# sota-zk-labs/zkp-implementation

Measured on AMD Instinct MI355X. Metric: G1 MSM scalar-muls/sec, higher is better.
Workload: dtype u32 (unsaturated 28-bit-limb Montgomery, 381-bit Fq; 64-bit accumulate)

## Files before the change

zkp-implementation_amd/build.py:

```python
#!/usr/bin/env python3
import os
import subprocess
import sys

HERE = os.path.dirname(os.path.abspath(__file__))
SRC = os.path.join(HERE, "csrc")
OUT = os.path.join(HERE, "libzkp_hip.so")
SOURCES = ["api.hip", "selftest.hip"]
DEPS = ["api.hip", "ff.hpp", "fq28.hpp", "fq28_inv.hpp", "fr29.hpp", "fr29_mul2_asm.inc", "fq28_mul_asm.inc", "fq28_mul2x_asm.inc", "fq28_sqr_asm.inc", "fq28_mul2_asm.inc", "g1.hpp", "g1_28.hpp", "msm.hpp", "ntt.hpp", "ntt_plan.hpp", "ntt_host.inc", "plonk.hpp",
        "plonk_host.inc", "plonk_compile_host.inc", "ntt_sharded.inc", "fri.hpp", "fri_host.inc", "fri_fr.hpp", "transcript_host.hpp", "pairing_host.hpp", "verify_host.inc", "host_ff.hpp", "kzg_host.hpp", "host_threads.hpp", "knobs.hpp", "msm_plan.hpp", "glv.hpp", "g1_check.hpp", "g1_check_host.inc", "g1_ntt.hpp", "g1_ntt_plan.hpp", "g1_ntt_host.inc", "msm_host.inc", "nova.hpp", "nova_host.inc", "dev_res.hpp", "selftest.hpp", "selftest.hip",
        os.path.join("..", "..", "include", "zkp_hip.h")]


STAMP = OUT + ".srchash"


def source_hash():
    import hashlib
    h = hashlib.sha256()
    for d in DEPS:
        path = os.path.join(SRC, d)
        if os.path.exists(path):
            h.update(d.encode())
            h.update(open(path, "rb").read())
    return h.hexdigest()


def stale():
    if not os.path.exists(OUT) or not os.path.exists(STAMP):
        return True
    return open(STAMP).read().strip() != source_hash()


def build(force=False, verbose=False, defines=(), out=None):
    variant = out is not None
    if not variant and not force and not stale():
        return OUT
    hipcc = os.environ.get("HIPCC", "/opt/rocm/bin/hipcc")
    cmd = [hipcc, "--offload-arch=gfx950", "-O3", "-std=c++17", "-fPIC", "-shared",
           "-Wno-unused-result", "-pthread"] + [f"-D{d}" for d in defines] + [os.path.join(SRC, s) for s in SOURCES] + ["-o", out or OUT]
    if verbose:
        print(" ".join(cmd))
    subprocess.check_call(cmd)
    if not variant:
        with open(STAMP, "w") as f:
            f.write(source_hash())
    return out or OUT


if __name__ == "__main__":
    defs = [a[2:] for a in sys.argv[1:] if a.startswith("-D")]
    outs = [a[2:] for a in sys.argv[1:] if a.startswith("-o")]
    print(build(force="--force" in sys.argv, verbose=True, defines=defs, out=outs[0] if outs else None))
```

zkp-implementation_amd/csrc/api.hip:

```cpp
#include <hip/hip_runtime.h>

#include <algorithm>
#include <array>
#include <atomic>
#include <chrono>
#include <cstdio>
#include <cstdlib>
#include <cstring>
#include <condition_variable>
#include <functional>
#include <map>
#include <memory>
#include <mutex>
#include <new>
#include <string>
#include <thread>
#include <tuple>
#include <type_traits>
#include <vector>

#include "../../include/zkp_hip.h"
#include "host_ff.hpp"
#include "kzg_host.hpp"
#include "msm.hpp"
#include "g1_check.hpp"
#include "ntt.hpp"
#include "g1_ntt.hpp"
#include "plonk.hpp"
#include "nova.hpp"
#include "fri.hpp"
#include "fri_fr.hpp"
#include "selftest.hpp"
#include "transcript_host.hpp"
#include "pairing_host.hpp"

using namespace zkp;
using namespace zkp::host;

namespace {

thread_local std::string g_err;

int fail(int code, const std::string& msg) {
    g_err = msg;
    return code;
}

int on_exception() noexcept {
    try {
        throw;
    } catch (const std::bad_alloc&) {
        try { g_err = "host allocation failed"; } catch (...) {}
        return ZKP_E_NOMEM;
    } catch (const std::exception& e) {
        try { g_err = std::string("internal error: ") + e.what(); } catch (...) {}
        return ZKP_E_DEVICE;
    } catch (...) {
        try { g_err = "internal error: unknown exception"; } catch (...) {}
        return ZKP_E_DEVICE;
    }
}
#define ZKP_CATCH_INT catch (...) { return on_exception(); }

#define HIPCHK(expr)                                                                                        \
    do {                                                                                                    \
        hipError_t e_ = (expr);                                                                             \
        if (e_ != hipSuccess)                                                                               \
            return fail(e_ == hipErrorOutOfMemory ? ZKP_E_NOMEM : ZKP_E_DEVICE,                             \
                        std::string(#expr) + ": " + hipGetErrorString(e_));                                 \
    } while (0)
int hip_fail(hipError_t e, const std::string& what) {
    return fail(e == hipErrorOutOfMemory ? ZKP_E_NOMEM : ZKP_E_DEVICE, what + hipGetErrorString(e));
}
#define HIPCHK_BARE(expr)                            \
    do {                                             \
        hipError_t e_ = (expr);                      \
        if (e_ != hipSuccess) return hip_fail(e_, ""); \
    } while (0)
#define ZCHK(expr)             \
    do {                       \
        int r_ = (expr);       \
        if (r_ != ZKP_OK) return r_; \
    } while (0)

#include "host_threads.hpp"
#include "dev_res.hpp"
static_assert(ZKP_HOST_THREADS_E_DEVICE == ZKP_E_DEVICE && ZKP_HOST_THREADS_OK == ZKP_OK, "host_threads.hpp error codes");

class DeviceWorkers {
    struct W {
        std::thread th;
        std::mutex mu;
        std::condition_variable cv;
        const std::function<void()>* job = nullptr;
        bool busy = false, quit = false;
    };
    std::mutex run_mu;
    std::vector<W*> ws;
    static void loop(W* w) {
        std::unique_lock<std::mutex> lk(w->mu);
        for (;;) {
            w->cv.wait(lk, [&] { return w->job != nullptr || w->quit; });
            if (w->quit) return;
            const std::function<void()>* j = w->job;
            lk.unlock();
            (*j)();
            lk.lock();
            w->job = nullptr;
            w->busy = false;
            w->cv.notify_all();
        }
    }

public:
    void run(const std::vector<std::function<void()>>& jobs) {
        std::lock_guard<std::mutex> one(run_mu);
        while (ws.size() < jobs.size()) {
            W* w = new W;
            w->th = std::thread(loop, w);
            ws.push_back(w);
        }
        for (size_t i = 0; i < jobs.size(); i++) {
            std::lock_guard<std::mutex> lk(ws[i]->mu);
            ws[i]->job = &jobs[i];
            ws[i]->busy = true;
            ws[i]->cv.notify_all();
        }
        for (size_t i = 0; i < jobs.size(); i++) {
            std::unique_lock<std::mutex> lk(ws[i]->mu);
            ws[i]->cv.wait(lk, [&] { return !ws[i]->busy; });
        }
    }
    void stop() {
        std::lock_guard<std::mutex> one(run_mu);
        for (W* w : ws) {
            {
                std::lock_guard<std::mutex> lk(w->mu);
                w->quit = true;
                w->cv.notify_all();
            }
            w->th.join();
            delete w;
        }
        ws.clear();
    }
};
DeviceWorkers g_workers;
void device_workers_stop() { g_workers.stop(); }

struct ProfRec {
    const char* name = nullptr;
    hipEvent_t a = nullptr;
    Event own_a, b;
    double host_ms = 0;
};
std::atomic<int> g_prof_on{0};
struct Ctx;
Ctx& ctx();
std::vector<ProfRec>& prof_records();
hipStream_t& prof_last_stream();

struct ProfScope {
    ProfRec rec;
    hipStream_t st;
    bool on;
    ProfScope(const char* name, hipStream_t s, bool chain = false) : st(s), on(false) {
        const int level = g_prof_on.load(std::memory_order_relaxed);
        on = name && (level == 1 || (level == 2 && std::strcmp(name, "msm_accumulate") == 0));
        if (!on) return;
        if (level == 2) chain = false;
        rec.name = name;
        std::vector<ProfRec>& recs = prof_records();
        if (chain && !recs.empty() && recs.back().b && prof_last_stream() == s) {
            rec.a = recs.back().b;
            if (rec.b.make(hipEventDefault) != hipSuccess) on = false;
            return;
        }
        if (rec.own_a.make(hipEventDefault) != hipSuccess || rec.b.make(hipEventDefault) != hipSuccess) { on = false; return; }
        rec.a = rec.own_a;
        (void)hipEventRecord(rec.a, st);
    }
    ~ProfScope() {
        if (!on) return;
        (void)hipEventRecord(rec.b, st);
        prof_records().push_back(std::move(rec));
        prof_last_stream() = st;
    }
};
void prof_host(const char* name, double ms) {
    if (g_prof_on.load(std::memory_order_relaxed) != 1) return;
    ProfRec r;
    r.name = name;
    r.host_ms = ms;
    prof_records().push_back(std::move(r));
}

enum { CLK_MSM_ACCUMULATE = 0, CLK_MAD_PROBE = 1, CLK_NTT_FR = 2, CLK_NTT_GL = 3, CLK_COUNT = 4 };
static const char* const kClkNames[CLK_COUNT] = {"msm_accumulate", "mad_probe", "ntt_fr_pass", "ntt_gl_pass"};

#include "ntt_host.inc"

struct Ctx {
    int slot = 0;
    int device = -1;
    std::mutex mu;
    Stream stream;
    Stream copy_stream;
    Stream sort_stream;
    Stream xstream;
    Event ws_event;
    hipStream_t ws_stream = nullptr;
    bool ws_pending = false;
    std::vector<ProfRec> prof;
    hipStream_t prof_last = nullptr;
    NttState<Fr> ntt_fr;
    NttState<Gl> ntt_gl;
    DevBuf ntt_scratch;
    DevBuf scalars, over;
    TypedBuf<uint32_t> digits, sorted, counts, start, perm, result;
    TypedBuf<uint2> entries;
    TypedBuf<uint4> pieces, buckets, parts, pyr1, odd0, odd1;
    PinnedBuf host_result;
    PinnedBuf fri_small;
    DevBuf fb_table;
    bool fb_ready = false;
    DevBuf g1_ntt_tw;
    bool g1_ntt_tw_ready = false;
    DevBuf tmp;
    Event copy_event;
    std::vector<Event> copy_events;
    Event ev_sort[2], ev_acc[2], ev_begin;
    DevBuf fri_arena, fri_meta;
    DevBuf clk;
    uint32_t tail_max_waves = 2048;
    DevBuf xchg_a, xchg_b;
    std::vector<Event> xev;
    bool peers_enabled = false;
    ~Ctx() {
        std::lock_guard<std::mutex> lk(mu);
        (void)hipSetDevice(device);
        (void)hipDeviceSynchronize();
    }
};

struct Runtime {
    std::mutex mu;
    std::vector<std::unique_ptr<Ctx>> slots;
    bool multi = false;
};
Runtime& g_rt = *new Runtime;

ClkRec* clk_record(int which) {
    if (!g_prof_on.load(std::memory_order_relaxed)) return nullptr;
    Ctx& c = ctx();
    if (!c.clk.p) {
        if (c.clk.ensure(sizeof(ClkRec) * CLK_COUNT) != ZKP_OK) return nullptr;
        if (hipMemset(c.clk.p, 0, sizeof(ClkRec) * CLK_COUNT) != hipSuccess) return nullptr;
    }
    return reinterpret_cast<ClkRec*>(c.clk.p) + which;
}
thread_local int t_slot = -1;
thread_local Ctx* t_cur = nullptr;
Ctx& ctx() { return *t_cur; }
std::vector<ProfRec>& prof_records() { return ctx().prof; }
hipStream_t& prof_last_stream() { return ctx().prof_last; }
template <class F> NttState<F>& ntt_state() { if constexpr (std::is_same<F, Fr>::value) return ctx().ntt_fr; else return ctx().ntt_gl; }
DevBuf& ntt_scratch() { return ctx().ntt_scratch; }

int create_slot_locked(int device);

struct CtxScope {
    Ctx* prev;
    std::unique_lock<std::mutex> lk;
    int rc = ZKP_OK;
    int restore_device = -1;
    explicit CtxScope(int slot) : prev(t_cur) {
        Ctx* c = nullptr;
        {
            std::lock_guard<std::mutex> g(g_rt.mu);
            if (g_rt.slots.empty()) {
                int dev = 0;
                if (hipGetDevice(&dev) != hipSuccess) dev = 0;
                rc = create_slot_locked(dev);
                if (rc != ZKP_OK) return;
            }
            const int s = slot >= 0 ? slot : (t_slot >= 0 ? t_slot : 0);
            if (s >= (int)g_rt.slots.size()) {
                rc = fail(ZKP_E_ARG, "device slot out of range (zkp_init_devices / zkp_set_device)");
                return;
            }
            c = g_rt.slots[(size_t)s].get();
        }
        lk = std::unique_lock<std::mutex>(c->mu);
        t_cur = c;
        int cur = -1;
        if (hipGetDevice(&cur) == hipSuccess && cur != c->device) restore_device = cur;
        if (cur != c->device && hipSetDevice(c->device) != hipSuccess) rc = fail(ZKP_E_DEVICE, "hipSetDevice failed");
    }
    ~CtxScope() {
        t_cur = prev;
        if (restore_device >= 0 && !prev) (void)hipSetDevice(restore_device);
    }
};
#define CTX_ENTER(slot)           \
    CtxScope ctx_scope_(slot);    \
    if (ctx_scope_.rc != ZKP_OK) return ctx_scope_.rc

struct WsOrder {
    hipStream_t st;
    explicit WsOrder(hipStream_t s) : st(s) {
        Ctx& c = ctx();
        if (c.ws_pending && c.ws_stream != st) (void)hipStreamWaitEvent(st, c.ws_event, 0);
    }
    ~WsOrder() {
        Ctx& c = ctx();
        if (c.ws_event.make(hipEventDisableTiming) != hipSuccess) {
            (void)hipStreamSynchronize(st);
            c.ws_pending = false;
            return;
        }
        (void)hipEventRecord(c.ws_event, st);
        c.ws_stream = st;
        c.ws_pending = true;
    }
};

template <class K>
int allow_big_lds(K kernel) {
    HIPCHK(hipFuncSetAttribute(reinterpret_cast<const void*>(kernel), hipFuncAttributeMaxDynamicSharedMemorySize,
                               160 * 1024));
    return ZKP_OK;
}

template <class F>
int ntt_host_entry(uint64_t* data, unsigned log_n, int inverse, const uint64_t* coset) {
    if (!data) return fail(ZKP_E_ARG, "data is null");
    if (log_n > 32) return fail(ZKP_E_ARG, "log_n > 32");
    CTX_ENTER(-1);
    WsOrder ord(nullptr);
    const size_t bytes = sizeof(F) << log_n;
    ZCHK(ctx().tmp.ensure(bytes));
    HIPCHK(hipMemcpyAsync(ctx().tmp.p, data, bytes, hipMemcpyHostToDevice, nullptr));
    ZCHK(run_ntt<F>(reinterpret_cast<F*>(ctx().tmp.p), log_n, 1, inverse, coset, nullptr));
    HIPCHK(hipMemcpyAsync(data, ctx().tmp.p, bytes, hipMemcpyDeviceToHost, nullptr));
    HIPCHK(hipStreamSynchronize(nullptr));
    return ZKP_OK;
}

}

struct zkp_bases {
    DevBuf d_xy;
    TypedBuf<uint8_t> d_inf;
    size_t n = 0;
    int device = 0;
    int slot = 0;
    std::vector<std::unique_ptr<zkp_bases>> shards;
    std::vector<size_t> shard_off;
    uint32_t pre_c = 0;
    uint32_t pre_planes = 0;
    uint32_t pre_req = 0;
    uint16_t pre_off[36] = {0};
    uint32_t pre_glv = 0;
};

namespace {

#include "msm_host.inc"

int ensure_fixed_base_table(hipStream_t st) {
    if (ctx().fb_ready) return ZKP_OK;
    static const uint64_t gx[6] = {0xfb3af00adb22c6bbULL, 0x6c55e83ff97a1aefULL, 0xa14e3a3f171bac58ULL,
                                   0xc3688c4f9774b905ULL, 0x2695638c4fa9ac0fULL, 0x17f1d3a73197d794ULL};
    static const uint64_t gy[6] = {0x0caa232946c5e7e1ULL, 0xd03cc744a2888ae4ULL, 0x00db18cb2c04b3edULL,
                                   0xfcf5e095d5d00af6ULL, 0xa09e30ed741d8ae4ULL, 0x08b3f481e3aaa0f1ULL};
    HXyzz base{HFq::load(gx).to_mont(), HFq::load(gy).to_mont(), HFq::one(), HFq::one()};
    const int NW = 32, ND = 255;
    std::vector<HXyzz> pts((size_t)NW * ND);
    for (int w = 0; w < NW; w++) {
        pts[(size_t)w * ND] = base;
        for (int d = 1; d < ND; d++) pts[(size_t)w * ND + d] = pts[(size_t)w * ND + d - 1].add(base);
        base = pts[(size_t)w * ND + ND - 1].add(base);
    }
    std::vector<uint64_t> tab(pts.size() * 12);
    std::vector<uint8_t> inf(pts.size());
    batch_to_affine(pts.data(), pts.size(), tab.data(), inf.data());
    ZCHK(ctx().fb_table.ensure(tab.size() * 8));
    HIPCHK(hipMemcpyAsync(ctx().fb_table.p, tab.data(), tab.size() * 8, hipMemcpyHostToDevice, st));
    HIPCHK(hipStreamSynchronize(st));
    ctx().fb_ready = true;
    return ZKP_OK;
}

}

extern "C" {

int zkp_abi_version(void) { return 1; }

void zkp_profile_enable(int on) { g_prof_on.store(on == 2 ? 2 : on != 0 ? 1 : 0); }
void zkp_profile_reset(void) {
    std::lock_guard<std::mutex> g(g_rt.mu);
    for (const auto& c : g_rt.slots) {
        std::lock_guard<std::mutex> lk(c->mu);
        c->prof.clear();
        if (c->clk.p) {
            int prev = 0;
            const bool restore = hipGetDevice(&prev) == hipSuccess && prev != c->device;
            if (restore) (void)hipSetDevice(c->device);
            (void)hipDeviceSynchronize();
            (void)hipMemset(c->clk.p, 0, sizeof(ClkRec) * CLK_COUNT);
            if (restore) (void)hipSetDevice(prev);
        }
    }
}
struct DeviceRestore {
    int dev = -1;
    DeviceRestore() { if (hipGetDevice(&dev) != hipSuccess) dev = -1; }
    ~DeviceRestore() { if (dev >= 0) (void)hipSetDevice(dev); }
};
int zkp_profile_clock_read(const char* name, uint64_t* cycles, uint64_t* ref_ticks, uint64_t* waves) try {
    if (!name || !cycles || !ref_ticks || !waves) return fail(ZKP_E_ARG, "null argument");
    int which = -1;
    for (int i = 0; i < CLK_COUNT; i++)
        if (std::strcmp(name, kClkNames[i]) == 0) which = i;
    if (which < 0) return fail(ZKP_E_ARG, "no clock stamps under this name (msm_accumulate, mad_probe, ntt_fr_pass, ntt_gl_pass)");
    std::lock_guard<std::mutex> g(g_rt.mu);
    *cycles = *ref_ticks = *waves = 0;
    DeviceRestore restore;
    for (const auto& c : g_rt.slots) {
        std::lock_guard<std::mutex> lk(c->mu);
        if (!c->clk.p) continue;
        ClkRec r;
        HIPCHK(hipSetDevice(c->device));
        HIPCHK(hipDeviceSynchronize());
        HIPCHK(hipMemcpy(&r, reinterpret_cast<ClkRec*>(c->clk.p) + which, sizeof r, hipMemcpyDeviceToHost));
        *cycles += r.cycles;
        *ref_ticks += r.ref;
        *waves += r.waves;
    }
    return ZKP_OK;
} ZKP_CATCH_INT

int zkp_probe_mad_rate(unsigned launches, double* lane_mads_per_s, double* clock_mhz, double* ms_per_launch) try {
    if (!lane_mads_per_s || !clock_mhz || !ms_per_launch) return fail(ZKP_E_ARG, "null argument");
    if (launches == 0 || launches > 1000) return fail(ZKP_E_ARG, "launches must be in 1..1000");
    CTX_ENTER(-1);
    WsOrder ord(nullptr);
    hipDeviceProp_t prop;
    HIPCHK(hipGetDeviceProperties(&prop, ctx().device));
    const unsigned blocks = (unsigned)prop.multiProcessorCount * 8;
    ZCHK(ctx().tmp.ensure((size_t)blocks * 256 * 4 + sizeof(ClkRec)));
    uint32_t* out = reinterpret_cast<uint32_t*>(ctx().tmp.p);
    ClkRec* rec = reinterpret_cast<ClkRec*>(out + (size_t)blocks * 256);
    HIPCHK(hipMemsetAsync(rec, 0, sizeof(ClkRec), nullptr));
    Event e0, e1;
    ZCHK(e0.ensure(hipEventDefault));
    ZCHK(e1.ensure(hipEventDefault));
    hipLaunchKernelGGL(mad_rate_probe_kernel, dim3(blocks), dim3(256), 0, nullptr, out, 7u, (ClkRec*)nullptr);
    HIPCHK(hipEventRecord(e0, nullptr));
    for (unsigned i = 0; i < launches; i++)
        hipLaunchKernelGGL(mad_rate_probe_kernel, dim3(blocks), dim3(256), 0, nullptr, out, 9u + i, rec);
    HIPCHK(hipEventRecord(e1, nullptr));
    HIPCHK(hipGetLastError());
    HIPCHK(hipEventSynchronize(e1));
    float ms = 0;
    HIPCHK(hipEventElapsedTime(&ms, e0, e1));
    ClkRec r;
    HIPCHK(hipMemcpy(&r, rec, sizeof r, hipMemcpyDeviceToHost));
    const double mads = (double)launches * blocks * 256.0 * MAD_PROBE_ITERS * MAD_PROBE_CHAINS;
    *lane_mads_per_s = mads / (ms * 1e-3);
    *clock_mhz = r.ref ? 100.0 * (double)r.cycles / (double)r.ref : 0.0;
    *ms_per_launch = ms / launches;
    return ZKP_OK;
} ZKP_CATCH_INT
int zkp_profile_read(const char* name, double* total_ms, uint64_t* count) try {
    if (!name || !total_ms || !count) return fail(ZKP_E_ARG, "null argument");
    std::lock_guard<std::mutex> g(g_rt.mu);
    double tot = 0;
    uint64_t cnt = 0;
    DeviceRestore restore;
    for (const auto& c : g_rt.slots) {
        std::lock_guard<std::mutex> lk(c->mu);
        HIPCHK(hipSetDevice(c->device));
        for (ProfRec& r : c->prof) {
            if (std::strcmp(r.name, name) != 0) continue;
            if (r.a) {
                HIPCHK(hipEventSynchronize(r.b));
                float ms = 0;
                HIPCHK(hipEventElapsedTime(&ms, r.a, r.b));
                tot += ms;
            } else {
                tot += r.host_ms;
            }
            cnt++;
        }
    }
    *total_ms = tot;
    *count = cnt;
    return ZKP_OK;
} ZKP_CATCH_INT
const char* zkp_last_error(void) { return g_err.c_str(); }

}

namespace {

int create_slot_locked(int device) {
    int count = 0;
    if (hipGetDeviceCount(&count) != hipSuccess || count == 0) return fail(ZKP_E_DEVICE, "no HIP device visible");
    if (device < 0 || device >= count) return fail(ZKP_E_ARG, "device index out of range");
    hipDeviceProp_t prop;
    HIPCHK(hipGetDeviceProperties(&prop, device));
    if (std::strncmp(prop.gcnArchName, "gfx950", 6) != 0)
        return fail(ZKP_E_DEVICE, std::string("device is ") + prop.gcnArchName + ", this library is built for gfx950 only");
    HIPCHK(hipSetDevice(device));
    ZCHK(allow_big_lds((ntt_pass_strided<Fr, NttOps<Fr>::LOG_T>)));
    ZCHK(allow_big_lds((ntt_pass_strided<Fr, NttOps<Fr>::LOG_T - 1>)));
    ZCHK(allow_big_lds((ntt_pass_strided<Fr, NttOps<Fr>::LOG_T - 2>)));
    ZCHK(allow_big_lds((ntt_pass_strided<Gl, NttOps<Gl>::LOG_T>)));
    ZCHK(allow_big_lds(ntt_pass_last<Fr>));
    ZCHK(allow_big_lds(ntt_pass_last<Gl>));
    ZCHK(allow_big_lds(msm_partscatter_kernel<PS_TILE_BIG>));
    ZCHK(allow_big_lds(msm_partscatter_kernel<PS_TILE_MID>));
    ZCHK(allow_big_lds(msm_partscatter_kernel<PS_TILE_SMALL>));
    ZCHK(allow_big_lds(fri_tail_kernel<FriGl>));
    ZCHK(allow_big_lds(fri_tail_kernel<FriFr>));
    auto c = std::make_unique<Ctx>();
    c->device = device;
    c->slot = (int)g_rt.slots.size();
    {
        int per_cu = 0;
        uint32_t cap = (uint32_t)prop.multiProcessorCount * 4 * 2;
        if (hipOccupancyMaxActiveBlocksPerMultiprocessor(&per_cu, msm_pyramid_tail_kernel, (int)PYR_TAIL_THREADS, 0) == hipSuccess && per_cu > 0)
            cap = std::min<uint32_t>(cap, (uint32_t)per_cu * (uint32_t)prop.multiProcessorCount * (PYR_TAIL_THREADS / 64));
        else
            (void)hipGetLastError();
        c->tail_max_waves = std::max<uint32_t>(cap, 4);
    }
    if (c->stream.make(hipStreamNonBlocking) != hipSuccess) return fail(ZKP_E_DEVICE, "hipStreamCreate failed");
    g_rt.slots.push_back(std::move(c));
    return ZKP_OK;
}

}

extern "C" {

int zkp_init(int device) try {
    std::lock_guard<std::mutex> g(g_rt.mu);
    if (!g_rt.slots.empty()) return ZKP_OK;
    if (device < 0 && hipGetDevice(&device) != hipSuccess) device = 0;
    return create_slot_locked(device);
} ZKP_CATCH_INT

int zkp_init_devices(const int* devices, int n_devices) try {
    if (n_devices < 0 || n_devices > 64) return fail(ZKP_E_ARG, "n_devices out of range");
    std::lock_guard<std::mutex> g(g_rt.mu);
    std::vector<int> want;
    if (n_devices == 0 || !devices) {
        int count = 0;
        if (hipGetDeviceCount(&count) != hipSuccess || count == 0) return fail(ZKP_E_DEVICE, "no HIP device visible");
        const int n = n_devices ? n_devices : count;
        if (n > count) return fail(ZKP_E_ARG, "more devices requested than visible");
        for (int i = 0; i < n; i++) want.push_back(i);
    } else {
        want.assign(devices, devices + n_devices);
    }
    if (!g_rt.slots.empty()) {
        bool same = g_rt.slots.size() == want.size();
        for (size_t i = 0; same && i < want.size(); i++) same = g_rt.slots[i]->device == want[i];
        return same ? ZKP_OK : fail(ZKP_E_ARG, "library already initialised with another device list (zkp_shutdown first)");
    }
    for (int d : want) {
        const int rc = create_slot_locked(d);
        if (rc != ZKP_OK) {
            g_rt.slots.clear();
            return rc;
        }
    }
    g_rt.multi = g_rt.slots.size() > 1;
    return ZKP_OK;
} ZKP_CATCH_INT

int zkp_device_count(void) {
    std::lock_guard<std::mutex> g(g_rt.mu);
    return (int)g_rt.slots.size();
}

int zkp_set_device(int slot) try {
    if (slot < -1) return fail(ZKP_E_ARG, "slot must be -1 (default) or a slot index");
    {
        std::lock_guard<std::mutex> g(g_rt.mu);
        if (slot >= 0 && !g_rt.slots.empty() && slot >= (int)g_rt.slots.size()) return fail(ZKP_E_ARG, "device slot out of range");
    }
    t_slot = slot;
    return ZKP_OK;
} ZKP_CATCH_INT

void zkp_shutdown(void) {
    device_workers_stop();
    std::lock_guard<std::mutex> g(g_rt.mu);
    g_rt.slots.clear();
    g_rt.multi = false;
}

}

namespace {

int bases_alloc(size_t n, bool with_inf, zkp_bases** out) {
    std::unique_ptr<zkp_bases> b(new (std::nothrow) zkp_bases());
    if (!b) return fail(ZKP_E_NOMEM, "host allocation failed");
    b->n = n;
    b->device = ctx().device;
    b->slot = ctx().slot;
    HIPCHK_BARE(b->d_xy.grow(std::max<size_t>(128 * n, 128)));
    if (with_inf) HIPCHK_BARE(b->d_inf.grow(std::max<size_t>(n, 1)));
    *out = b.release();
    return ZKP_OK;
}

void shard_range(size_t n, size_t i, size_t k, size_t* lo, size_t* hi) {
    const size_t base = n / k, rem = n % k;
    *lo = i * base + std::min(i, rem);
    *hi = *lo + base + (i < rem ? 1 : 0);
}

int bases_create_single(int slot, const uint64_t* xy, const uint8_t* is_inf, size_t n, zkp_bases** out) {
    CTX_ENTER(slot);
    hipStream_t st = g_rt.multi ? ctx().stream : nullptr;
    WsOrder ord(st);
    zkp_bases* b = nullptr;
    ZCHK(bases_alloc(n, is_inf != nullptr, &b));
    hipError_t e = hipSuccess;
    if (n) {
        int rc = ctx().tmp.ensure(96 * n);
        if (rc != ZKP_OK) {
            zkp_g1_bases_destroy(b);
            return rc;
        }
        e = hipMemcpyAsync(ctx().tmp.p, xy, 96 * n, hipMemcpyHostToDevice, st);
        if (e == hipSuccess) {
            hipLaunchKernelGGL(g1_to_internal_kernel, dim3((unsigned)((n + MSM_THREADS - 1) / MSM_THREADS)),
                               dim3(MSM_THREADS), 0, st, reinterpret_cast<const uint4*>(ctx().tmp.p), (uint64_t)n,
                               static_cast<uint4*>(b->d_xy.p));
            e = hipGetLastError();
        }
        if (e == hipSuccess && is_inf) e = hipMemcpyAsync(b->d_inf.p, is_inf, n, hipMemcpyHostToDevice, st);
        if (e == hipSuccess) e = hipStreamSynchronize(st);
    }
    if (e != hipSuccess) {
        zkp_g1_bases_destroy(b);
        return fail(ZKP_E_DEVICE, hipGetErrorString(e));
    }
    *out = b;
    return ZKP_OK;
}

int for_each_shard(const zkp_bases* b, const std::function<int(size_t)>& fn) {
    const size_t k = b->shards.size();
    std::vector<int> rc(k, ZKP_OK);
    std::vector<std::string> msg(k);
    std::vector<std::function<void()>> jobs(k);
    for (size_t i = 0; i < k; i++)
        jobs[i] = [&, i] {
            try {
                rc[i] = fn(i);
            } catch (...) {
                rc[i] = on_exception();
            }
            if (rc[i] != ZKP_OK) msg[i] = g_err;
        };
    g_workers.run(jobs);
    for (size_t i = 0; i < k; i++)
        if (rc[i] != ZKP_OK)
            return fail(rc[i], "device slot " + std::to_string(b->shards[i] ? b->shards[i]->slot : (int)i) + ": " + msg[i]);
    return ZKP_OK;
}

unsigned auto_window_bits(size_t n) {
    if (n < 64) return 0;
    return n >= (1u << 22) ? 22 : n >= (1u << 19) ? 20 : n > (1u << 13) ? 16 : n > (1u << 11) ? 14 : 12;
}

int precompute_single(zkp_bases* b, unsigned window_bits, bool glv, bool check_only = false) {
    if (b->pre_c && (b->pre_glv != 0) != glv)
        return fail(ZKP_E_ARG, b->pre_glv ? "bases already expanded for the endomorphism-split MSM (zkp_g1_bases_precompute_glv)"
                                          : "bases already expanded for whole scalars (zkp_g1_bases_precompute)");
    if (window_bits == 0) {
        if (b->pre_c || b->n < 64) return ZKP_OK;
        window_bits = auto_window_bits(b->n);
    }
    if (window_bits < 9 || window_bits > MSM_MAX_WINDOW_BITS) return fail(ZKP_E_ARG, "window_bits must be 0 (automatic) or in 9.." + std::to_string(MSM_MAX_WINDOW_BITS));
    if (b->pre_c) return b->pre_req == window_bits ? ZKP_OK : fail(ZKP_E_ARG, "bases already expanded with another width");
    CTX_ENTER(b->slot);
    hipStream_t st = g_rt.multi ? ctx().stream : nullptr;
    WsOrder ord(st);
    if (!b->n) return ZKP_OK;
    const MsmSlices sl = msm_slice_offsets(glv ? GlvParams::COVER_BITS : 256, window_bits, (uint32_t)knob_int(KNOB_MSM_BALANCE_FROM));
    const uint32_t planes = sl.planes, cmax = sl.widest;
    SliceOffsets so;
    static_assert(sizeof so.off == sizeof sl.off, "SliceOffsets");
    std::memcpy(so.off, sl.off, sizeof so.off);
    DevBuf p;
    {
        const size_t need = 128 * (size_t)planes * b->n;
        size_t free_b = 0, total_b = 0;
        if (hipMemGetInfo(&free_b, &total_b) != hipSuccess) free_b = total_b = 0, (void)hipGetLastError();
        const size_t budget = std::min<size_t>(free_b ? free_b : ~(size_t)0, (size_t)knob_int(KNOB_SRS_EXPAND_MAX_BYTES));
        auto too_large = [&](const char* why) {
            return fail(ZKP_E_NOMEM, "SRS expansion does not fit (" + std::string(why) + "): " + std::to_string(planes) + " planes x " +
                                         std::to_string(b->n) + " points x 128 B = " + std::to_string(need) + " bytes, " +
                                         std::to_string(free_b) + " of " + std::to_string(total_b) +
                                         " bytes free on the device; the bases stay unexpanded (per-window MSM), or shard the SRS over "
                                         "more devices (zkp_init_devices)");
        };
        if (need > budget) return too_large(need > free_b && free_b ? "device memory" : "ZKP_SRS_EXPAND_MAX_BYTES");
        if (check_only) return ZKP_OK;
        if (p.ensure(need) != ZKP_OK) {
            (void)hipGetLastError();
            return too_large("hipMalloc");
        }
    }
    hipError_t e = hipMemcpyAsync(p.p, b->d_xy.p, 128 * b->n, hipMemcpyDeviceToDevice, st);
    const uint64_t step = std::min<uint64_t>(b->n, 1ull << 18);
    if (e == hipSuccess && ctx().tmp.ensure(192 * (size_t)planes * step) != ZKP_OK) e = hipErrorOutOfMemory;
    for (uint64_t off = 0; e == hipSuccess && off < b->n; off += step) {
        const uint64_t cnt = std::min<uint64_t>(step, b->n - off);
        hipLaunchKernelGGL(g1_expand_planes_kernel, dim3((unsigned)((cnt + MSM_THREADS - 1) / MSM_THREADS)), dim3(MSM_THREADS),
                           0, st, static_cast<uint4*>(p.p), reinterpret_cast<uint4*>(ctx().tmp.p), off, cnt,
                           (uint64_t)b->n, planes, so);
        e = hipGetLastError();
    }
    if (e == hipSuccess) e = hipStreamSynchronize(st);
    if (e != hipSuccess)
        return fail(e == hipErrorOutOfMemory ? ZKP_E_NOMEM : ZKP_E_DEVICE, std::string("SRS expansion: ") + hipGetErrorString(e));
    b->d_xy = std::move(p);
    b->pre_c = cmax;
    b->pre_req = window_bits;
    b->pre_planes = planes;
    b->pre_glv = glv ? 1u : 0u;
    std::memcpy(b->pre_off, so.off, sizeof so.off);
    return ZKP_OK;
}

int unexpand_single(zkp_bases* b) {
    if (!b->pre_c) return ZKP_OK;
    CTX_ENTER(b->slot);
    hipStream_t st = g_rt.multi ? ctx().stream : nullptr;
    WsOrder ord(st);
    DevBuf p;
    ZCHK(p.ensure(128 * std::max<size_t>(b->n, 1)));
    hipError_t e = hipMemcpyAsync(p.p, b->d_xy.p, 128 * b->n, hipMemcpyDeviceToDevice, st);
    if (e == hipSuccess) e = hipStreamSynchronize(st);
    if (e != hipSuccess) return fail(ZKP_E_DEVICE, hipGetErrorString(e));
    b->d_xy = std::move(p);
    b->pre_c = b->pre_req = b->pre_planes = b->pre_glv = 0;
    return ZKP_OK;
}

int slot_of_device_pointer(const void* d_ptr, int* slot) {
    *slot = t_slot;
    hipPointerAttribute_t attr;
    if (hipPointerGetAttributes(&attr, d_ptr) != hipSuccess) return ZKP_OK;
    std::lock_guard<std::mutex> g(g_rt.mu);
    if (*slot >= 0 && *slot < (int)g_rt.slots.size() && g_rt.slots[(size_t)*slot]->device != attr.device) *slot = -1;
    for (size_t i = 0; *slot < 0 && i < g_rt.slots.size(); i++)
        if (g_rt.slots[i]->device == attr.device) *slot = (int)i;
    if (*slot < 0 && !g_rt.slots.empty()) return fail(ZKP_E_ARG, "device pointer belongs to a device the library was not initialised on");
    return ZKP_OK;
}

}

extern "C" {

int zkp_g1_bases_create(const uint64_t* xy, const uint8_t* is_inf, size_t n, zkp_bases** out) try {
    if (!out || (n && !xy)) return fail(ZKP_E_ARG, "null argument");
    size_t nslots = 0;
    {
        std::lock_guard<std::mutex> g(g_rt.mu);
        nslots = g_rt.slots.size();
    }
    if (nslots <= 1 || t_slot >= 0) return bases_create_single(t_slot >= 0 ? t_slot : 0, xy, is_inf, n, out);
    zkp_bases* c = new (std::nothrow) zkp_bases();
    if (!c) return fail(ZKP_E_NOMEM, "host allocation failed");
    c->n = n;
    c->slot = -1;
    c->shards.resize(nslots);
    c->shard_off.assign(nslots, 0);
    for (size_t i = 0; i < nslots; i++) {
        size_t hi = 0;
        shard_range(n, i, nslots, &c->shard_off[i], &hi);
    }
    const int rc = for_each_shard(c, [&](size_t i) {
        size_t lo = 0, hi = 0;
        shard_range(n, i, nslots, &lo, &hi);
        zkp_bases* s = nullptr;
        const int r = bases_create_single((int)i, xy + 12 * lo, is_inf ? is_inf + lo : nullptr, hi - lo, &s);
        c->shards[i].reset(s);
        return r;
    });
    if (rc != ZKP_OK) {
        zkp_g1_bases_destroy(c);
        return rc;
    }
    *out = c;
    return ZKP_OK;
} ZKP_CATCH_INT

int zkp_g1_bases_create_dev(const void* d_xy, const uint8_t* d_is_inf, size_t n, void* stream, zkp_bases** out) try {
    if (!out || (n && !d_xy)) return fail(ZKP_E_ARG, "null argument");
    int slot = t_slot;
    if (n) ZCHK(slot_of_device_pointer(d_xy, &slot));
    CTX_ENTER(slot);
    hipStream_t st = reinterpret_cast<hipStream_t>(stream);
    WsOrder ord(st);
    zkp_bases* b = nullptr;
    ZCHK(bases_alloc(n, d_is_inf != nullptr, &b));
    hipError_t e = hipSuccess;
    if (n) {
        hipLaunchKernelGGL(g1_to_internal_kernel, dim3((unsigned)((n + MSM_THREADS - 1) / MSM_THREADS)), dim3(MSM_THREADS),
                           0, st, reinterpret_cast<const uint4*>(d_xy), (uint64_t)n, static_cast<uint4*>(b->d_xy.p));
        e = hipGetLastError();
    }
    if (e == hipSuccess && n && d_is_inf) e = hipMemcpyAsync(b->d_inf.p, d_is_inf, n, hipMemcpyDeviceToDevice, st);
    if (e == hipSuccess) e = hipStreamSynchronize(st);
    if (e != hipSuccess) {
        zkp_g1_bases_destroy(b);
        return fail(ZKP_E_DEVICE, hipGetErrorString(e));
    }
    *out = b;
    return ZKP_OK;
} ZKP_CATCH_INT

static int precompute_any(zkp_bases* b, unsigned window_bits, bool glv) {
    if (!b) return fail(ZKP_E_ARG, "null argument");
    if (b->shards.empty()) return precompute_single(b, window_bits, glv);
    size_t nmax = 0, expanded = 0;
    for (const auto& sh : b->shards) nmax = std::max(nmax, sh->n), expanded += sh->pre_c ? 1 : 0;
    for (const auto& sh : b->shards)
        if (sh->pre_c && (sh->pre_glv != 0) != glv) return precompute_single(sh.get(), window_bits, glv, true);
    if (window_bits == 0) {
        if (expanded == b->shards.size() || !(window_bits = auto_window_bits(nmax))) return ZKP_OK;
        if (expanded) window_bits = b->shards[0]->pre_req ? b->shards[0]->pre_req : window_bits;
    }
    ZCHK(for_each_shard(b, [&](size_t i) { return precompute_single(b->shards[i].get(), window_bits, glv, true); }));
    std::vector<uint8_t> was(b->shards.size());
    for (size_t i = 0; i < b->shards.size(); i++) was[i] = b->shards[i]->pre_c ? 1 : 0;
    const int rc = for_each_shard(b, [&](size_t i) { return precompute_single(b->shards[i].get(), window_bits, glv); });
    if (rc != ZKP_OK) {
        const std::string why = zkp_last_error();
        bool mixed = false;
        for (size_t i = 0; i < b->shards.size(); i++)
            if (!was[i] && b->shards[i]->pre_c && unexpand_single(b->shards[i].get()) != ZKP_OK) mixed = true;
        return fail(rc, why + (mixed ? " -- and a finished chunk could not be rolled back: the handle is expanded in part (still usable)"
                                     : " -- every chunk is back to the plain points"));
    }
    return ZKP_OK;
}

int zkp_g1_bases_precompute(zkp_bases* b, unsigned window_bits) try { return precompute_any(b, window_bits, false); } ZKP_CATCH_INT

int zkp_g1_bases_precompute_glv(zkp_bases* b, unsigned window_bits) try { return precompute_any(b, window_bits, true); } ZKP_CATCH_INT

int zkp_g1_bases_expansion(const zkp_bases* b, zkp_bases_expansion* out) try {
    if (!b || !out) return fail(ZKP_E_ARG, "null argument");
    const zkp_bases* s = b->shards.empty() ? b : b->shards[0].get();
    if (!s) return fail(ZKP_E_ARG, "empty handle");
    *out = zkp_bases_expansion{};
    if (!s->pre_c) return ZKP_OK;
    out->window_bits = s->pre_req;
    out->planes = s->pre_planes;
    out->glv = s->pre_glv;
    out->slices = s->pre_planes * (s->pre_glv ? 2u : 1u);
    out->widest_slice_bits = s->pre_c;
    if (b->shards.empty()) out->bytes = 128 * (size_t)s->pre_planes * s->n;
    for (const auto& sh : b->shards) out->bytes += sh->pre_c ? 128 * (size_t)sh->pre_planes * sh->n : 0;
    return ZKP_OK;
} ZKP_CATCH_INT

size_t zkp_g1_bases_len(const zkp_bases* b) { return b ? b->n : 0; }

int zkp_g1_bases_info(const zkp_bases* b, unsigned* window_bits, unsigned* slices) try {
    if (!b || !window_bits || !slices) return fail(ZKP_E_ARG, "null argument");
    const zkp_bases* s = b->shards.empty() ? b : b->shards[0].get();
    if (!s) return fail(ZKP_E_ARG, "empty handle");
    *window_bits = s->pre_req;
    *slices = s->pre_c ? s->pre_planes * (s->pre_glv ? 2u : 1u) : 0;
    return ZKP_OK;
} ZKP_CATCH_INT

void zkp_g1_bases_destroy(zkp_bases* b) {
    if (!b) return;
    for (auto& s : b->shards) zkp_g1_bases_destroy(s.release());
    DeviceRestore restore;
    (void)hipSetDevice(b->device);
    delete b;
}

}

namespace {

const char* const kShardedDev = "bases are sharded over several devices: device-pointer entries take single-device bases "
                                "(zkp_set_device + zkp_g1_bases_create*); use zkp_msm_g1 with host scalars";

int msm_host_scalars(const zkp_bases* bases, const uint64_t* scalars, size_t n, HXyzz* r) {
    CTX_ENTER(bases->slot);
    hipStream_t st = g_rt.multi ? ctx().stream : nullptr;
    WsOrder ord(st);
    if (n > bases->n) return fail(ZKP_E_SIZE, "more scalars than bases (kzg/src/scheme.rs:86)");
    *r = HXyzz::infinity();
    if (!n) return ZKP_OK;
    ZCHK(ctx().scalars.ensure(32 * n));
    const Fr* d_sc = reinterpret_cast<const Fr*>(ctx().scalars.p);
    const bool shared = bases->pre_c != 0;
    if (shared && n >= (1u << 19)) {
        ZCHK(ctx().copy_stream.ensure(hipStreamNonBlocking));
        ZCHK(ctx().copy_event.ensure(hipEventDisableTiming));
        const MsmFeed feed{scalars, ctx().copy_stream, ctx().copy_event, msm_feed_ranges(n)};
        return msm_partial_batch(bases, &d_sc, 1, n, st, r, &feed);
    }
    HIPCHK(hipMemcpyAsync(ctx().scalars.p, scalars, 32 * n, hipMemcpyHostToDevice, st));
    return msm_partial(bases, d_sc, n, st, r);
}

int msm_over_shards(const zkp_bases* bases, size_t n, const std::function<int(size_t, size_t, size_t, HXyzz*)>& body, HXyzz* r) {
    std::vector<HXyzz> part(bases->shards.size(), HXyzz::infinity());
    ZCHK(for_each_shard(bases, [&](size_t i) {
        const size_t lo = bases->shard_off[i], have = bases->shards[i]->n;
        if (lo >= n || !have) return (int)ZKP_OK;
        return body(i, lo, std::min(have, n - lo), &part[i]);
    }));
    *r = HXyzz::infinity();
    for (const HXyzz& p : part) *r = r->add(p);
    return ZKP_OK;
}

int msm_host_scalars_any(const zkp_bases* bases, const uint64_t* scalars, size_t n, HXyzz* r) {
    if (bases->shards.empty()) return msm_host_scalars(bases, scalars, n, r);
    if (n > bases->n) return fail(ZKP_E_SIZE, "more scalars than bases (kzg/src/scheme.rs:86)");
    return msm_over_shards(bases, n, [&](size_t i, size_t lo, size_t len, HXyzz* part) {
        return msm_host_scalars(bases->shards[i].get(), scalars + 4 * lo, len, part);
    }, r);
}

}

extern "C" {

int zkp_msm_g1_partial_dev(const zkp_bases* bases, const void* d_scalars, size_t n, void* stream, uint64_t out_xyzz[24]) try {
    if (!bases || !out_xyzz || (n && !d_scalars)) return fail(ZKP_E_ARG, "null argument");
    if (!bases->shards.empty()) return fail(ZKP_E_ARG, kShardedDev);
    CTX_ENTER(bases->slot);
    WsOrder ord(reinterpret_cast<hipStream_t>(stream));
    HXyzz r;
    ZCHK(msm_partial(bases, reinterpret_cast<const Fr*>(d_scalars), n, reinterpret_cast<hipStream_t>(stream), &r));
    r.store(out_xyzz);
    return ZKP_OK;
} ZKP_CATCH_INT

int zkp_msm_g1_dev(const zkp_bases* bases, const void* d_scalars, size_t n, void* stream, uint64_t out_xy[12],
                   uint8_t* out_is_inf) try {
    if (!bases || !out_xy || !out_is_inf || (n && !d_scalars)) return fail(ZKP_E_ARG, "null argument");
    if (!bases->shards.empty()) return fail(ZKP_E_ARG, kShardedDev);
    CTX_ENTER(bases->slot);
    WsOrder ord(reinterpret_cast<hipStream_t>(stream));
    HXyzz r;
    ZCHK(msm_partial(bases, reinterpret_cast<const Fr*>(d_scalars), n, reinterpret_cast<hipStream_t>(stream), &r));
    r.to_affine(out_xy, out_is_inf);
    return ZKP_OK;
} ZKP_CATCH_INT

int zkp_msm_g1(const zkp_bases* bases, const uint64_t* scalars, size_t n, uint64_t out_xy[12], uint8_t* out_is_inf) try {
    if (!bases || !out_xy || !out_is_inf || (n && !scalars)) return fail(ZKP_E_ARG, "null argument");
    HXyzz r;
    ZCHK(msm_host_scalars_any(bases, scalars, n, &r));
    r.to_affine(out_xy, out_is_inf);
    return ZKP_OK;
} ZKP_CATCH_INT

int zkp_g1_bases_shard_count(const zkp_bases* b) { return !b ? 0 : b->shards.empty() ? 1 : (int)b->shards.size(); }

int zkp_g1_bases_shard(const zkp_bases* b, size_t i, int* slot, int* device, size_t* offset, size_t* len) try {
    if (!b || !slot || !device || !offset || !len) return fail(ZKP_E_ARG, "null argument");
    if (i >= (size_t)zkp_g1_bases_shard_count(b)) return fail(ZKP_E_ARG, "chunk index out of range");
    const zkp_bases* s = b->shards.empty() ? b : b->shards[i].get();
    *slot = s->slot;
    *device = s->device;
    *offset = b->shards.empty() ? 0 : b->shard_off[i];
    *len = s->n;
    return ZKP_OK;
} ZKP_CATCH_INT

static int order_after_producer(hipStream_t st, void* ready_event) {
    if (ready_event) HIPCHK(hipStreamWaitEvent(st, reinterpret_cast<hipEvent_t>(ready_event), 0));
    else HIPCHK(hipDeviceSynchronize());
    return ZKP_OK;
}

int zkp_msm_g1_sharded_dev_after(const zkp_bases* bases, const void* const* d_scalars, void* const* ready_events, size_t n,
                                 uint64_t out_xy[12], uint8_t* out_is_inf) try {
    if (!bases || !out_xy || !out_is_inf || (n && !d_scalars)) return fail(ZKP_E_ARG, "null argument");
    if (n > bases->n) return fail(ZKP_E_SIZE, "more scalars than bases (kzg/src/scheme.rs:86)");
    HXyzz acc = HXyzz::infinity();
    if (bases->shards.empty()) {
        if (n) {
            if (!d_scalars[0]) return fail(ZKP_E_ARG, "null scalar pointer");
            CTX_ENTER(bases->slot);
            hipStream_t st = g_rt.multi ? ctx().stream : nullptr;
            ZCHK(order_after_producer(st, ready_events ? ready_events[0] : nullptr));
            WsOrder ord(st);
            ZCHK(msm_partial(bases, reinterpret_cast<const Fr*>(d_scalars[0]), n, st, &acc));
        }
    } else {
        for (size_t i = 0; i < bases->shards.size(); i++)
            if (bases->shard_off[i] < n && bases->shards[i]->n && !d_scalars[i]) return fail(ZKP_E_ARG, "null scalar pointer for a chunk in use");
        ZCHK(msm_over_shards(bases, n, [&](size_t i, size_t, size_t len, HXyzz* part) {
            const zkp_bases* sh = bases->shards[i].get();
            CTX_ENTER(sh->slot);
            ZCHK(order_after_producer(ctx().stream, ready_events ? ready_events[i] : nullptr));
            WsOrder ord(ctx().stream);
            return msm_partial(sh, reinterpret_cast<const Fr*>(d_scalars[i]), len, ctx().stream, part);
        }, &acc));
    }
    acc.to_affine(out_xy, out_is_inf);
    return ZKP_OK;
} ZKP_CATCH_INT

int zkp_msm_g1_sharded_dev(const zkp_bases* bases, const void* const* d_scalars, size_t n, uint64_t out_xy[12],
                           uint8_t* out_is_inf) {
    return zkp_msm_g1_sharded_dev_after(bases, d_scalars, nullptr, n, out_xy, out_is_inf);
}

int zkp_msm_g1_partial(const zkp_bases* bases, const uint64_t* scalars, size_t n, uint64_t out_xyzz[24]) try {
    if (!bases || !out_xyzz || (n && !scalars)) return fail(ZKP_E_ARG, "null argument");
    HXyzz r;
    ZCHK(msm_host_scalars_any(bases, scalars, n, &r));
    r.store(out_xyzz);
    return ZKP_OK;
} ZKP_CATCH_INT

int zkp_msm_g1_batch_dev(const zkp_bases* bases, const void* const* d_scalars, size_t count, size_t n, void* stream,
                         uint64_t* out_xy, uint8_t* out_is_inf) try {
    if (!bases || (count && (!d_scalars || !out_xy || !out_is_inf))) return fail(ZKP_E_ARG, "null argument");
    if (!bases->shards.empty()) return fail(ZKP_E_ARG, kShardedDev);
    CTX_ENTER(bases->slot);
    WsOrder ord(reinterpret_cast<hipStream_t>(stream));
    std::vector<HXyzz> r(count);
    ZCHK(msm_partial_batch(bases, reinterpret_cast<const Fr* const*>(d_scalars), count, n, reinterpret_cast<hipStream_t>(stream),
                           r.data()));
    batch_to_affine(r.data(), count, out_xy, out_is_inf);
    return ZKP_OK;
} ZKP_CATCH_INT

int zkp_g1_xyzz_sum(const uint64_t* partials, size_t count, uint64_t out_xy[12], uint8_t* out_is_inf) try {
    if ((count && !partials) || !out_xy || !out_is_inf) return fail(ZKP_E_ARG, "null argument");
    HXyzz acc = HXyzz::infinity();
    for (size_t i = 0; i < count; i++) acc = acc.add(HXyzz::load(partials + 24 * i));
    acc.to_affine(out_xy, out_is_inf);
    return ZKP_OK;
} ZKP_CATCH_INT

int zkp_kzg_commit(const zkp_bases* srs, const uint64_t* coeffs, size_t len, uint64_t out_xy[12], uint8_t* out_is_inf) try {
    if (!srs || !out_xy || !out_is_inf || (len && !coeffs)) return fail(ZKP_E_ARG, "null argument");
    KzgScheme scheme(srs);
    KzgCommitment cm;
    int rc = scheme.commit(coeffs, len, &cm);
    if (rc == ZKP_E_SIZE && g_err.empty()) g_err = "SRS shorter than the polynomial (kzg/src/scheme.rs:86)";
    if (rc != ZKP_OK) return rc;
    std::memcpy(out_xy, cm.p.xy, 96);
    *out_is_inf = cm.p.infinity;
    return ZKP_OK;
} ZKP_CATCH_INT

int kzg_open_device(const zkp_bases* srs, const uint64_t* coeffs, size_t len, const uint64_t z[4], uint64_t out_xy[12],
                    uint8_t* out_is_inf, uint64_t out_eval[4]);

int zkp_kzg_open(const zkp_bases* srs, const uint64_t* coeffs, size_t len, const uint64_t z[4], uint64_t out_xy[12],
                 uint8_t* out_is_inf, uint64_t out_eval[4]) try {
    if (!srs || !out_xy || !out_is_inf || !out_eval || !z || (len && !coeffs)) return fail(ZKP_E_ARG, "null argument");
    if (len == 0) return fail(ZKP_E_ARG, "open of an empty polynomial (kzg/src/scheme.rs:112 expects at least 1)");
    if (len >= 4096) return kzg_open_device(srs, coeffs, len, z, out_xy, out_is_inf, out_eval);
    KzgScheme scheme(srs);
    KzgOpening op;
    int rc = scheme.open(coeffs, len, z, &op);
    if (rc != ZKP_OK) return rc;
    std::memcpy(out_xy, op.p.xy, 96);
    *out_is_inf = op.p.infinity;
    op.eval.store(out_eval);
    return ZKP_OK;
} ZKP_CATCH_INT

int zkp_g1_mul(const uint64_t base_xy[12], uint8_t base_is_inf, const uint64_t scalar[4], uint64_t out_xy[12],
               uint8_t* out_is_inf) try {
    if (!base_xy || !scalar || !out_xy || !out_is_inf) return fail(ZKP_E_ARG, "null argument");
    HFr k = HFr::load(scalar).from_mont();
    HXyzz r = HXyzz::from_affine(base_xy, base_is_inf != 0).mul(k.l);
    r.to_affine(out_xy, out_is_inf);
    return ZKP_OK;
} ZKP_CATCH_INT

static int fixed_base_mul_locked(const void* d_scalars, size_t n, void* d_out_xy, uint8_t* d_out_is_inf, hipStream_t st) {
    ZCHK(ensure_fixed_base_table(st));
    hipLaunchKernelGGL(g1_fixed_base_kernel, dim3((unsigned)((n + MSM_THREADS - 1) / MSM_THREADS)), dim3(MSM_THREADS), 0,
                       st, reinterpret_cast<const Fr*>(d_scalars), (uint64_t)n,
                       reinterpret_cast<const uint4*>(ctx().fb_table.p), reinterpret_cast<uint4*>(d_out_xy), d_out_is_inf);
    HIPCHK(hipGetLastError());
    return ZKP_OK;
}

int zkp_g1_fixed_base_mul_dev(const void* d_scalars, size_t n, void* d_out_xy, uint8_t* d_out_is_inf, void* stream) try {
    if (n && (!d_scalars || !d_out_xy)) return fail(ZKP_E_ARG, "null argument");
    CTX_ENTER(-1);
    if (!n) return ZKP_OK;
    WsOrder ord(reinterpret_cast<hipStream_t>(stream));
    return fixed_base_mul_locked(d_scalars, n, d_out_xy, d_out_is_inf, reinterpret_cast<hipStream_t>(stream));
} ZKP_CATCH_INT

int zkp_selftest_fq_inverse_dev(const void* d_in, size_t n, int form, void* d_out, void* stream) try {
    if (n && (!d_in || !d_out)) return fail(ZKP_E_ARG, "null argument");
    if (form != 0 && form != 1) return fail(ZKP_E_ARG, "form must be 0 (12 x u32, radix 2^384) or 1 (14 x 28 bit + 2 pad words, radix 2^392)");
    CTX_ENTER(-1);
    if (!n) return ZKP_OK;
    hipLaunchKernelGGL(fq_inverse_selftest_kernel, dim3((unsigned)((n + MSM_THREADS - 1) / MSM_THREADS)), dim3(MSM_THREADS), 0,
                       reinterpret_cast<hipStream_t>(stream), reinterpret_cast<const uint32_t*>(d_in), reinterpret_cast<uint32_t*>(d_out),
                       (uint64_t)n, form);
    HIPCHK(hipGetLastError());
    return ZKP_OK;
} ZKP_CATCH_INT

namespace {
unsigned selftest_grid(size_t lanes) { return (unsigned)((lanes + ST_THREADS - 1) / ST_THREADS); }
int selftest_args(const void* d_in, size_t n, const void* d_out) {
    if (n && (!d_in || !d_out)) return fail(ZKP_E_ARG, "null argument");
    if (d_in && d_in == d_out) return fail(ZKP_E_ARG, "d_out must not be d_in");
    if (n > (size_t)1 << 24) return fail(ZKP_E_SIZE, "a self-test takes at most 2^24 cases");
    return ZKP_OK;
}
}

int zkp_selftest_fq28_dev(int op, const void* d_in, size_t n, void* d_out, void* stream) try {
    ZCHK(selftest_args(d_in, n, d_out));
    if (op < 0 || op >= ST_FQ28_OPS) return fail(ZKP_E_ARG, "unknown Fq28 self-test operation");
    CTX_ENTER(-1);
    if (!n) return ZKP_OK;
    selftest_fq28_launch(op, selftest_grid(n), reinterpret_cast<hipStream_t>(stream), d_in, d_out, (uint64_t)n);
    HIPCHK(hipGetLastError());
    return ZKP_OK;
} ZKP_CATCH_INT

int zkp_selftest_fr29_dev(int op, const void* d_in, size_t n, void* d_out, void* stream) try {
    ZCHK(selftest_args(d_in, n, d_out));
    if (op < 0 || op >= ST_FR29_OPS) return fail(ZKP_E_ARG, "unknown Fr29 self-test operation");
    CTX_ENTER(-1);
    if (!n) return ZKP_OK;
    selftest_fr29_launch(op, selftest_grid(n), reinterpret_cast<hipStream_t>(stream), d_in, d_out, (uint64_t)n);
    HIPCHK(hipGetLastError());
    return ZKP_OK;
} ZKP_CATCH_INT

int zkp_selftest_fp_dev(int field, int op, const void* d_in, size_t n, void* d_out, void* stream) try {
    ZCHK(selftest_args(d_in, n, d_out));
    if (field != 0 && field != 1) return fail(ZKP_E_ARG, "field must be 0 (Fq, 12 words) or 1 (Fr, 8 words)");
    if (op < 0 || op >= ST_FP_OPS) return fail(ZKP_E_ARG, "unknown Fp self-test operation");
    CTX_ENTER(-1);
    if (!n) return ZKP_OK;
    selftest_fp_launch(field, op, selftest_grid(n), reinterpret_cast<hipStream_t>(stream), d_in, d_out, (uint64_t)n);
    HIPCHK(hipGetLastError());
    return ZKP_OK;
} ZKP_CATCH_INT

int zkp_selftest_gl_dev(int op, const void* d_in, size_t n, void* d_out, void* stream) try {
    ZCHK(selftest_args(d_in, n, d_out));
    if (op < 0 || op >= ST_GL_OPS) return fail(ZKP_E_ARG, "unknown Goldilocks self-test operation");
    CTX_ENTER(-1);
    if (!n) return ZKP_OK;
    selftest_gl_launch(op, selftest_grid(n), reinterpret_cast<hipStream_t>(stream), d_in, d_out, (uint64_t)n);
    HIPCHK(hipGetLastError());
    return ZKP_OK;
} ZKP_CATCH_INT

int zkp_selftest_g1_dev(int op, const void* d_a, const void* d_b, size_t n, size_t stride, void* d_out, void* d_flag, void* stream) try {
    if (op < 0 || op >= ST_G1_OPS) return fail(ZKP_E_ARG, "unknown G1 self-test operation");
    const bool in_place = op == ST_G1_ADD_INPLACE || op == ST_G1_ADD_INPLACE_CHAIN || op == ST_G1_ADD_QUAD_INPLACE;
    const bool planes = op >= ST_G1_ADD_STREAM;
    if (n && ((!d_a && !in_place) || !d_b || !d_out || !d_flag)) return fail(ZKP_E_ARG, "null argument");
    if (d_b && d_b == d_out) return fail(ZKP_E_ARG, "d_out must not be d_b");
    if ((op == ST_G1_ADD_STREAM || op == ST_G1_ADD_STREAM_CHAIN) && d_a == d_out) return fail(ZKP_E_ARG, "the streaming add does not alias: use the in-place operation");
    if (n > (size_t)1 << 24) return fail(ZKP_E_SIZE, "a self-test takes at most 2^24 cases");
    if (planes && stride < n) return fail(ZKP_E_ARG, "stride below the number of cases");
    CTX_ENTER(-1);
    if (!n) return ZKP_OK;
    const bool quad = op == ST_G1_ADD_QUAD || op == ST_G1_ADD_QUAD_INPLACE;
    selftest_g1_launch(op, selftest_grid(quad ? 4 * n : n), reinterpret_cast<hipStream_t>(stream), d_a, d_b, d_out, d_flag, (uint64_t)n,
                       (uint64_t)stride);
    HIPCHK(hipGetLastError());
    return ZKP_OK;
} ZKP_CATCH_INT

int zkp_selftest_glv_split_dev(const void* d_scalars, size_t n, void* d_out, void* stream) try {
    ZCHK(selftest_args(d_scalars, n, d_out));
    CTX_ENTER(-1);
    if (!n) return ZKP_OK;
    selftest_glv_split_launch(selftest_grid(n), reinterpret_cast<hipStream_t>(stream), d_scalars, d_out, (uint64_t)n);
    HIPCHK(hipGetLastError());
    return ZKP_OK;
} ZKP_CATCH_INT

int zkp_srs_g1(const uint64_t secret[4], size_t n, uint64_t* out_xy) try {
    if (!secret || (n && !out_xy)) return fail(ZKP_E_ARG, "null argument");
    if (!n) return ZKP_OK;
    std::vector<uint64_t> pw(4 * n);
    HFr s = HFr::load(secret), cur = HFr::one();
    for (size_t i = 0; i < n; i++) {
        cur.store(&pw[4 * i]);
        cur = cur * s;
    }
    CTX_ENTER(-1);
    WsOrder ord(nullptr);
    ZCHK(ctx().tmp.ensure(32 * n + 96 * n));
    char* d = reinterpret_cast<char*>(ctx().tmp.p);
    HIPCHK(hipMemcpy(d, pw.data(), 32 * n, hipMemcpyHostToDevice));
    ZCHK(fixed_base_mul_locked(d, n, d + 32 * n, nullptr, nullptr));
    HIPCHK(hipMemcpy(out_xy, d + 32 * n, 96 * n, hipMemcpyDeviceToHost));
    return ZKP_OK;
} ZKP_CATCH_INT

}
bool ntt_should_shard(unsigned log_n);
int ntt_fr_sharded_host(uint64_t* data, unsigned log_n, int inverse, const uint64_t* coset);
extern "C" {
int zkp_ntt_fr(uint64_t* data, unsigned log_n, int inverse, const uint64_t* coset) try {
    if (ntt_should_shard(log_n)) return ntt_fr_sharded_host(data, log_n, inverse, coset);
    return ntt_host_entry<Fr>(data, log_n, inverse, coset);
} ZKP_CATCH_INT
int zkp_ntt_goldilocks(uint64_t* data, unsigned log_n, int inverse, const uint64_t* coset) try {
    return ntt_host_entry<Gl>(data, log_n, inverse, coset);
} ZKP_CATCH_INT
int zkp_ntt_fr_dev(void* d_data, unsigned log_n, size_t batch, int inverse, const uint64_t* coset, void* stream) try {
    if (!d_data) return fail(ZKP_E_ARG, "data is null");
    CTX_ENTER(-1);
    WsOrder ord(reinterpret_cast<hipStream_t>(stream));
    return run_ntt<Fr>(reinterpret_cast<Fr*>(d_data), log_n, batch, inverse, coset, reinterpret_cast<hipStream_t>(stream));
} ZKP_CATCH_INT
int zkp_ntt_goldilocks_dev(void* d_data, unsigned log_n, size_t batch, int inverse, const uint64_t* coset, void* stream) try {
    if (!d_data) return fail(ZKP_E_ARG, "data is null");
    CTX_ENTER(-1);
    WsOrder ord(reinterpret_cast<hipStream_t>(stream));
    return run_ntt<Gl>(reinterpret_cast<Gl*>(d_data), log_n, batch, inverse, coset, reinterpret_cast<hipStream_t>(stream));
} ZKP_CATCH_INT

int zkp_ntt_fr_twiddle_dev(void* d_data, size_t rows, size_t cols, size_t row0, unsigned log_n, int inverse, void* stream) try {
    if (!d_data) return fail(ZKP_E_ARG, "data is null");
    if (log_n > 32 || log_n == 0) return fail(ZKP_E_ARG, "log_n out of range");
    if ((uint64_t)(row0 + rows - 1) * (cols - 1) >= (1ull << log_n) && rows && cols)
        return fail(ZKP_E_ARG, "twiddle exponent (row0 + rows - 1) * (cols - 1) must stay below n");
    CTX_ENTER(-1);
    if (!rows || !cols) return ZKP_OK;
    hipStream_t st = reinterpret_cast<hipStream_t>(stream);
    WsOrder ord(st);
    PowTab<Fr> tab;
    HFr w = fr_root_of_unity(log_n);
    ZCHK(get_coset_tables<Fr>(log_n, inverse ? 1 : 0, w.l, HFr::one(), &tab, st));
    const uint64_t total = (uint64_t)rows * cols;
    hipLaunchKernelGGL(twiddle_rows_kernel<Fr>, dim3((unsigned)((total + 255) / 256)), dim3(256), 0, st,
                       reinterpret_cast<Fr*>(d_data), (uint64_t)rows, (uint64_t)cols, (uint64_t)row0, tab);
    HIPCHK(hipGetLastError());
    return ZKP_OK;
} ZKP_CATCH_INT

int zkp_ntt_fr_axis0_dev(const void* d_in, void* d_out, unsigned log_len, size_t cols, int inverse, unsigned tw_log_n,
                         size_t tw_col0, void* stream) try {
    if (!d_in || !d_out) return fail(ZKP_E_ARG, "data is null");
    CTX_ENTER(-1);
    hipStream_t st = reinterpret_cast<hipStream_t>(stream);
    WsOrder ord(st);
    return run_ntt_axis0<Fr>(reinterpret_cast<const Fr*>(d_in), reinterpret_cast<Fr*>(d_out), log_len, cols, inverse, tw_log_n,
                             (uint64_t)tw_col0, st);
} ZKP_CATCH_INT

int zkp_ntt_fr_layout_dev(const void* d_in, void* d_out, unsigned log_n, size_t batch, int inverse, const zkp_ntt_layout* in_layout,
                          const zkp_ntt_layout* out_layout, unsigned tw_log_n, size_t tw_row0, void* stream) try {
    if (!d_in || !d_out) return fail(ZKP_E_ARG, "data is null");
    if (log_n > 32) return fail(ZKP_E_ARG, "log_n > 32");
    NttRemap rin, rout;
    const zkp_ntt_layout* ls[2] = {in_layout, out_layout};
    NttRemap* rs[2] = {&rin, &rout};
    for (int i = 0; i < 2; i++) {
        std::memset(rs[i], 0, sizeof(NttRemap));
        if (!ls[i]) continue;
        if (ls[i]->lo_bits + ls[i]->mid_bits > log_n || ls[i]->lo_bits < 2)
            return fail(ZKP_E_ARG, "layout: lo_bits must be >= 2 (16-byte runs of four elements) and lo_bits + mid_bits <= log_n");
        rs[i]->on = 1;
        rs[i]->lo_bits = ls[i]->lo_bits;
        rs[i]->mid_bits = ls[i]->mid_bits;
        rs[i]->mid_stride = ls[i]->mid_stride;
        rs[i]->hi_stride = ls[i]->hi_stride;
        rs[i]->batch_stride = ls[i]->batch_stride;
    }
    if (d_in == d_out && (in_layout || out_layout))
        return fail(ZKP_E_ARG, "a transform with a gathered or scattered layout cannot run in place");
    CTX_ENTER(-1);
    hipStream_t st = reinterpret_cast<hipStream_t>(stream);
    WsOrder ord(st);
    NttIo io;
    io.in_remap = in_layout ? &rin : nullptr;
    io.out_remap = out_layout ? &rout : nullptr;
    io.tw_log_n = tw_log_n;
    io.tw_row0 = (uint64_t)tw_row0;
    return run_ntt<Fr>(reinterpret_cast<const Fr*>(d_in), reinterpret_cast<Fr*>(d_out), log_n, batch, inverse, nullptr, st, &io);
} ZKP_CATCH_INT

int zkp_poly_mul_fr(const uint64_t* a, size_t la, const uint64_t* b, size_t lb, uint64_t* out) try {
    if (la == 0 || lb == 0) return ZKP_OK;
    if (!a || !b || !out) return fail(ZKP_E_ARG, "null argument");
    const size_t lo = la + lb - 1;
    unsigned log_n = 0;
    while (((size_t)1 << log_n) < lo) log_n++;
    const size_t n = (size_t)1 << log_n;
    CTX_ENTER(-1);
    WsOrder ord(nullptr);
    ZCHK(ctx().tmp.ensure(2 * 32 * n));
    char* d = reinterpret_cast<char*>(ctx().tmp.p);
    HIPCHK(hipMemsetAsync(d, 0, 2 * 32 * n, nullptr));
    HIPCHK(hipMemcpyAsync(d, a, 32 * la, hipMemcpyHostToDevice, nullptr));
    HIPCHK(hipMemcpyAsync(d + 32 * n, b, 32 * lb, hipMemcpyHostToDevice, nullptr));
    ZCHK(run_ntt<Fr>(reinterpret_cast<Fr*>(d), log_n, 2, 0, nullptr, nullptr));
    hipLaunchKernelGGL(pointwise_mul_kernel<Fr>, dim3((unsigned)((n + 255) / 256)), dim3(256), 0, nullptr,
                       reinterpret_cast<const Fr*>(d), reinterpret_cast<const Fr*>(d + 32 * n), reinterpret_cast<Fr*>(d),
                       (uint64_t)n);
    HIPCHK(hipGetLastError());
    ZCHK(run_ntt<Fr>(reinterpret_cast<Fr*>(d), log_n, 1, 1, nullptr, nullptr));
    HIPCHK(hipMemcpyAsync(out, d, 32 * lo, hipMemcpyDeviceToHost, nullptr));
    HIPCHK(hipStreamSynchronize(nullptr));
    return ZKP_OK;
} ZKP_CATCH_INT

}

#include "ntt_sharded.inc"
#include "plonk_host.inc"
#include "plonk_compile_host.inc"
#include "fri_host.inc"
#include "verify_host.inc"
#include "g1_check_host.inc"
#include "g1_ntt_host.inc"
#include "nova_host.inc"
```

zkp-implementation_amd/csrc/host_threads.hpp:

```cpp
#pragma once
#include <atomic>
#include <chrono>
#include <condition_variable>
#include <functional>
#include <mutex>
#include <thread>
#include <vector>

#ifndef ZKP_HOST_THREADS_E_DEVICE
#define ZKP_HOST_THREADS_E_DEVICE (-3)
#endif
#ifndef ZKP_HOST_THREADS_OK
#define ZKP_HOST_THREADS_OK 0
#endif

class HostPool {
    std::mutex run_mu;
    std::mutex mu;
    std::condition_variable cv, cv_done;
    const std::function<void(size_t)>* fn = nullptr;
    size_t next = 0, total = 0, finished = 0;
    bool started = false;
    std::atomic<bool> posted{false};
    std::chrono::steady_clock::time_point warm_until{};
    void worker() {
        std::unique_lock<std::mutex> lk(mu);
        for (;;) {
            cv.wait(lk, [&] { return (fn != nullptr && next < total) || std::chrono::steady_clock::now() < warm_until; });
            if (!(fn != nullptr && next < total)) {
                const auto until = warm_until;
                lk.unlock();
                while (!posted.load(std::memory_order_acquire) && std::chrono::steady_clock::now() < until) __builtin_ia32_pause();
                lk.lock();
                if (!(fn != nullptr && next < total)) {
                    if (std::chrono::steady_clock::now() >= warm_until) warm_until = {};
                    continue;
                }
            }
            const size_t i = next++;
            const std::function<void(size_t)>* f = fn;
            lk.unlock();
            (*f)(i);
            lk.lock();
            if (++finished == total) cv_done.notify_one();
        }
    }

public:
    void run(const std::function<void(size_t)>& f, size_t n) {
        std::lock_guard<std::mutex> one(run_mu);
        std::unique_lock<std::mutex> lk(mu);
        if (!started) {
            started = true;
            for (int i = 0; i < 3; i++) std::thread([this] { worker(); }).detach();
        }
        fn = &f;
        next = 0;
        total = n;
        finished = 0;
        warm_until = {};
        posted.store(true, std::memory_order_release);
        cv.notify_all();
        while (next < total) {
            const size_t i = next++;
            lk.unlock();
            f(i);
            lk.lock();
            ++finished;
        }
        cv_done.wait(lk, [&] { return finished == total; });
        fn = nullptr;
        posted.store(false, std::memory_order_release);
        warm_until = {};
    }
    void warm(std::chrono::microseconds how_long) {
        std::unique_lock<std::mutex> lk(mu, std::try_to_lock);
        if (!lk.owns_lock() || !started) return;
        warm_until = std::chrono::steady_clock::now() + how_long;
        cv.notify_all();
    }
};
HostPool& host_pool() {
    static HostPool* pool = new HostPool;
    return *pool;
}

class Uploader {
    std::mutex mu;
    std::condition_variable cv, cv_done;
    std::function<int()> job;
    bool pending = false, running = false, started = false;
    int rc = ZKP_HOST_THREADS_OK;
    void worker() {
        std::unique_lock<std::mutex> lk(mu);
        for (;;) {
            cv.wait(lk, [&] { return pending; });
            pending = false;
            running = true;
            std::function<int()> f = std::move(job);
            lk.unlock();
            int r;
            try {
                r = f();
            } catch (...) {
                r = ZKP_HOST_THREADS_E_DEVICE;
            }
            lk.lock();
            rc = r;
            running = false;
            cv_done.notify_all();
        }
    }

public:
    void submit(std::function<int()> f) {
        std::unique_lock<std::mutex> lk(mu);
        if (!started) {
            started = true;
            std::thread([this] { worker(); }).detach();
        }
        job = std::move(f);
        pending = true;
        cv.notify_one();
    }
    int wait() {
        std::unique_lock<std::mutex> lk(mu);
        cv_done.wait(lk, [&] { return !pending && !running; });
        return rc;
    }
};
Uploader& uploader(int slot) {
    static std::mutex mu;
    static std::vector<Uploader*> all;
    std::lock_guard<std::mutex> lk(mu);
    if (slot < 0) slot = 0;
    while (all.size() <= (size_t)slot) all.push_back(new Uploader);
    return *all[(size_t)slot];
}

class RangeUpload {
    std::atomic<uint64_t> issued_{0};
    std::atomic<int> rc_{ZKP_HOST_THREADS_OK}, go_{0};
    std::vector<uint64_t> lens_;
    Uploader* up_ = nullptr;

public:
    RangeUpload() = default;
    RangeUpload(const RangeUpload&) = delete;
    RangeUpload& operator=(const RangeUpload&) = delete;
    ~RangeUpload() { (void)join(); }
    template <class Prepare, class Issue>
    void submit(Uploader& up, std::vector<uint64_t> later, uint64_t first, Prepare prepare, Issue issue) {
        lens_ = std::move(later);
        up.submit([this, first, prepare, issue]() -> int {
            int rc = prepare();
            int go;
            while ((go = go_.load(std::memory_order_acquire)) == 0) __builtin_ia32_pause();
            if (go < 0) return ZKP_HOST_THREADS_OK;
            uint64_t o = first;
            for (size_t k = 0; rc == ZKP_HOST_THREADS_OK && k < lens_.size(); o += lens_[k++])
                if ((rc = issue(k, o, lens_[k])) == ZKP_HOST_THREADS_OK) issued_.store(k + 1, std::memory_order_release);
            if (rc != ZKP_HOST_THREADS_OK) rc_.store(rc, std::memory_order_release);
            return rc;
        });
        up_ = &up;
    }
    void release(bool ok) { go_.store(ok ? 1 : -1, std::memory_order_release); }
    bool wait_issued(uint64_t k) const {
        for (; issued_.load(std::memory_order_acquire) < k; __builtin_ia32_pause())
            if (rc_.load(std::memory_order_acquire) != ZKP_HOST_THREADS_OK) return false;
        return true;
    }
    int join() {
        if (!up_) return ZKP_HOST_THREADS_OK;
        int unreleased = 0;
        go_.compare_exchange_strong(unreleased, -1, std::memory_order_acq_rel);
        Uploader* up = up_;
        up_ = nullptr;
        return up->wait();
    }
};
```

zkp-implementation_amd/csrc/msm_host.inc:

```

#ifdef ZKP_MSM_CHECK
#define MSM_TRACE(stream, ridx, what) do { hipError_t e_ = hipStreamSynchronize(stream); fprintf(stderr, "ZKP_MSM_CHECK range %llu: %s done (%d)\n", (unsigned long long)(ridx), what, (int)e_); } while (0)
#else
#define MSM_TRACE(stream, ridx, what) do { } while (0)
#endif

struct MsmFeed {
    const uint64_t* h_scalars;
    hipStream_t copy_stream;
    hipEvent_t ev;
    MsmFeedRanges ranges;
};

struct RangeBuffers {
    uint32_t *sorted, *start, *perm;
    uint4* desc;
    uint32_t *over, *over_b, *over_off;
};

struct MsmPass {
    const MsmPlan& p;
    MsmGeom g;
    const zkp_bases* bases;
    const Fr* const* scalars;
    size_t count;
    const MsmFeed* feed;
    hipStream_t st, sst;
    Ctx& cx = ctx();
    const size_t W = p.g.nwin, nhi = p.sg.nhi;
    uint32_t *ptot, *pstart, *ghist, *gcur;
    uint4* result_out;
    uint32_t* result_flags;
    RangeUpload up;

    std::array<std::tuple<const char*, DevBuf*, size_t>, 14> buffers() {
        const MsmSizes& b = p.bytes;
        return {{{"digits", &cx.digits, b.digits}, {"sorted", &cx.sorted, b.sorted}, {"counts", &cx.counts, b.counts},
                 {"entries", &cx.entries, b.entries}, {"start", &cx.start, b.start}, {"perm", &cx.perm, b.perm}, {"over", &cx.over, b.over},
                 {"pieces", &cx.pieces, b.pieces}, {"buckets", &cx.buckets, b.buckets}, {"parts", &cx.parts, b.parts},
                 {"pyr1", &cx.pyr1, b.pyr1}, {"odd0", &cx.odd0, b.odd0}, {"odd1", &cx.odd1, b.odd1}, {"result", &cx.result, b.result}}};
    }
    int grow() {
        for (const auto& [name, buf, bytes] : buffers()) ZCHK(buf->ensure(bytes));
        ZCHK(cx.host_result.ensure(p.bytes.host_result, hipHostMallocPortable | hipHostMallocMapped));
        ptot = cx.counts.get() + W * g.nchunk * nhi;
        pstart = ptot + W * nhi;
        ghist = pstart + W * (nhi + 1);
        gcur = ghist + W * 256;
        result_out = static_cast<uint4*>(cx.host_result.p);
        result_flags = reinterpret_cast<uint32_t*>(result_out + 16 * W * g.c);
        return ZKP_OK;
    }
    RangeBuffers range_buffers(size_t par) const {
        uint4* desc = reinterpret_cast<uint4*>(static_cast<char*>(cx.over.p) + par * p.over_bytes);
        uint32_t* over = reinterpret_cast<uint32_t*>(desc + W * p.desc_cap);
        return {cx.sorted.get() + par * W * p.g.n, cx.start.get() + par * W * (p.g.nb + 2), cx.perm.get() + par * W * p.g.nb, desc, over,
                over + 2 * W, over + 2 * W + W * p.over_cap};
    }
#ifdef ZKP_MSM_CHECK
    void dump(size_t n) {
        static bool once = false;
        if (once) return;
        once = true;
        auto show = [](const char* name, const void* q, size_t bytes) {
            fprintf(stderr, "ZKP_MSM_CHECK %-10s %p .. %p (%zu bytes)\n", name, q, static_cast<const char*>(q) + bytes, bytes);
        };
        show("bases", bases->d_xy.p, (size_t)bases->n * 128 * std::max(bases->pre_planes, 1u));
        show("scalars", scalars[0], 32 * n);
        for (const auto& [name, buf, bytes] : buffers()) show(name, buf->p, buf->cap);
        show("host_res", cx.host_result.p, cx.host_result.cap);
        fprintf(stderr, "ZKP_MSM_CHECK geometry: n %zu range %llu first %llu rest %llu entries %llu nb %u nchunk %u over_cap %u desc_cap %u run_limit %u piece %u\n",
                n, (unsigned long long)p.range, (unsigned long long)p.lens[0], (unsigned long long)p.lens.back(), (unsigned long long)p.g.n,
                p.g.nb, p.g.nchunk, p.over_cap, p.desc_cap, p.g.run_limit, p.g.piece);
    }
#endif

    int feed_first_range() {
        Fr* const dst = const_cast<Fr*>(scalars[0]);
        if (p.lens.size() > 1) {
            while (cx.copy_events.size() < p.lens.size() - 1) {
                Event e;
                ZCHK(e.ensure(hipEventDisableTiming));
                cx.copy_events.push_back(std::move(e));
            }
            up.submit(uploader(cx.slot), std::vector<uint64_t>(p.lens.begin() + 1, p.lens.end()), p.lens[0],
                      [device = cx.device] { return hipSetDevice(device) == hipSuccess ? (int)ZKP_OK : (int)ZKP_E_DEVICE; },
                      [dst, f = *feed, evs = cx.copy_events.data()](size_t k, uint64_t o, uint64_t l) {
                          const bool ok = hipMemcpyAsync(dst + o, f.h_scalars + 4 * o, 32 * l, hipMemcpyHostToDevice, f.copy_stream) == hipSuccess &&
                                          hipEventRecord(evs[k], f.copy_stream) == hipSuccess;
                          return ok ? (int)ZKP_OK : (int)ZKP_E_DEVICE;
                      });
        }
        hipError_t e1 = hipMemcpyAsync(dst, feed->h_scalars, 32 * p.lens[0], hipMemcpyHostToDevice, feed->copy_stream);
        if (e1 == hipSuccess) e1 = hipEventRecord(feed->ev, feed->copy_stream);
        up.release(e1 == hipSuccess);
        HIPCHK(e1);
        return ZKP_OK;
    }

    int walk() {
        if (p.overlap) {
            ZCHK(cx.sort_stream.ensure(hipStreamNonBlocking));
            for (Event* e : {&cx.ev_sort[0], &cx.ev_sort[1], &cx.ev_acc[0], &cx.ev_acc[1], &cx.ev_begin}) ZCHK(e->ensure(hipEventDisableTiming));
            sst = cx.sort_stream;
            HIPCHK(hipEventRecord(cx.ev_begin, st));
            HIPCHK(hipStreamWaitEvent(sst, cx.ev_begin, 0));
        }
        for (size_t ridx = 0, off = 0; ridx < p.lens.size(); off += p.lens[ridx++]) {
            const uint64_t len = p.lens[ridx];
            const size_t par = p.overlap ? (ridx & 1) : 0;
            const RangeBuffers rb = range_buffers(par);
            if (p.overlap && ridx >= 2) HIPCHK(hipStreamWaitEvent(sst, cx.ev_acc[par], 0));
            if (len != g.ns) {
                g.ns = len;
                g.n = (uint64_t)p.nwin1 * len;
                g.chunk = (g.n + g.nchunk - 1) / g.nchunk;
            }
            g.resume = off ? 1u : 0u;
            g.more = ridx + 1 < p.lens.size() ? 1u : 0u;
            if (feed) {
                if (ridx == 0)
                    ZCHK(feed_first_range());
                else if (!up.wait_issued(ridx))
                    return fail(ZKP_E_DEVICE, "upload of a scalar range failed");
                HIPCHK(hipStreamWaitEvent(sst, ridx == 0 ? feed->ev : cx.copy_events[ridx - 1], 0));
            }
            launch_sort(rb, off, ridx);
            if (p.overlap) {
                HIPCHK(hipEventRecord(cx.ev_sort[par], sst));
                HIPCHK(hipStreamWaitEvent(st, cx.ev_sort[par], 0));
            }
            launch_accumulate(rb, off, ridx);
            if (p.overlap) HIPCHK(hipEventRecord(cx.ev_acc[par], st));
        }
        return ZKP_OK;
    }

    template <int TILE> void launch_partscatter() {
        hipLaunchKernelGGL(msm_partscatter_kernel<TILE>, dim3(g.nchunk, g.nwin), dim3(1024), partscatter_lds_bytes(nhi, TILE), sst,
                           cx.digits.get(), g, p.sg, cx.counts.get(), pstart, cx.entries.get());
    }
    void launch_sort(const RangeBuffers& rb, uint64_t off, size_t ridx) {
        const SortGeom& sg = p.sg;
        {
            ProfScope ps("msm_digits", sst);
            DigitSources ds;
            for (size_t m = 0; m < count; m++) ds.scalars[m] = scalars[m] + off;
            hipLaunchKernelGGL(g.glv ? msm_digits_glv_kernel : msm_digits_kernel, dim3((unsigned)((g.ns + MSM_THREADS - 1) / MSM_THREADS), (unsigned)count), dim3(MSM_THREADS), 0,
                               sst, ds, bases->d_inf.p ? bases->d_inf.get() + off : nullptr, g, p.nwin1, cx.digits.get());
            MSM_TRACE(sst, ridx, "digits");
        }
        ProfScope ps("msm_sort", sst, true);
        hipLaunchKernelGGL(msm_parthist_kernel, dim3(g.nchunk, g.nwin), dim3(1024), 0, sst, cx.digits.get(), g, sg, cx.counts.get());
        MSM_TRACE(sst, ridx, "parthist");
        hipLaunchKernelGGL(msm_partprefix_kernel, dim3((sg.nhi + 63) / 64, g.nwin), dim3(1024), 0, sst, cx.counts.get(), g, sg, ptot);
        hipLaunchKernelGGL(msm_partstart_kernel, dim3(g.nwin), dim3(64), 0, sst, ptot, sg, pstart, ghist, cx.result.get());
        MSM_TRACE(sst, ridx, "partprefix + partstart");
        switch (partscatter_tile(sg.nhi)) {
            case PS_TILE_SMALL: launch_partscatter<PS_TILE_SMALL>(); break;
            case PS_TILE_MID: launch_partscatter<PS_TILE_MID>(); break;
            default: launch_partscatter<PS_TILE_BIG>(); break;
        }
        MSM_TRACE(sst, ridx, "partscatter");
        hipLaunchKernelGGL(msm_binsort_kernel, dim3(sg.nhi, g.nwin), dim3(1024), 0, sst, cx.entries.get(), g, sg, pstart, rb.start, rb.sorted, ghist);
        MSM_TRACE(sst, ridx, "binsort");
        hipLaunchKernelGGL(msm_rank_kernel, dim3((g.nb + 1023) / 1024, g.nwin), dim3(1024), 0, sst, rb.start, g, ghist, gcur, rb.perm);
        MSM_TRACE(sst, ridx, "rank");
        hipLaunchKernelGGL(msm_order_kernel, dim3(g.nwin), dim3(1024), 0, sst, rb.start, g, ghist, rb.perm, rb.over, rb.over_b, rb.over_off,
                           rb.desc, p.over_cap, p.desc_cap);
        MSM_TRACE(sst, ridx, "order");
    }

    void launch_accumulate(const RangeBuffers& rb, uint64_t off, size_t ridx) {
        ProfScope ps("msm_accumulate", st, true);
        const bool quad = !g.resume && !g.more && (uint64_t)g.n * g.nwin <= (1ull << 20);
        const uint32_t per_block = quad ? ACC_THREADS / 4 : ACC_THREADS;
        const uint32_t bucket_blocks = (uint32_t)((((uint64_t)g.nb << g.split_log) + per_block - 1) / per_block);
        const uint32_t extra_blocks = std::min<uint32_t>((p.desc_cap + per_block - 1) / per_block, 64);
        const dim3 grid((bucket_blocks + extra_blocks) * g.nwin);
        const uint4* xy = static_cast<const uint4*>(bases->d_xy.p) + off * 8;
        uint4 *buckets = cx.buckets.get(), *pieces = cx.pieces.get(), *parts = cx.parts.get(), *carry = cx.pyr1.get();
        if (quad)
            hipLaunchKernelGGL(msm_accumulate_quad_kernel, grid, dim3(ACC_THREADS), 0, st, xy, rb.sorted, rb.start, rb.perm, rb.over, rb.desc,
                               p.desc_cap, bucket_blocks, extra_blocks, g, buckets, pieces, parts, clk_record(CLK_MSM_ACCUMULATE));
        else
            hipLaunchKernelGGL(msm_accumulate_kernel, grid, dim3(ACC_THREADS), 0, st, xy, rb.sorted, rb.start, rb.perm, rb.over, rb.desc,
                               p.desc_cap, bucket_blocks, extra_blocks, g, buckets, pieces, parts, carry, clk_record(CLK_MSM_ACCUMULATE));
        MSM_TRACE(st, ridx, "accumulate");
        hipLaunchKernelGGL(msm_combine_kernel, dim3(std::min<uint32_t>(p.over_cap, 64), g.nwin), dim3(64), 0, st, rb.over, rb.over_b,
                           rb.over_off, p.over_cap, p.desc_cap, g, pieces, buckets, carry);
        MSM_TRACE(st, ridx, "combine");
        const uint64_t cap = (uint64_t)g.nwin * g.nb;
        const uint64_t lane_from = (uint64_t)knob_int(KNOB_FOLD_LANE_MIN);
        for (uint32_t t = 0; t < g.split_log; t++) {
            const unsigned pairs = 1u << (g.split_log - 1 - t), per = cap * pairs >= lane_from ? MSM_THREADS : MSM_THREADS / 4;
            hipLaunchKernelGGL(per == MSM_THREADS ? msm_fold_parts_lane_kernel : msm_fold_parts_kernel, dim3((unsigned)((cap + per - 1) / per), pairs),
                               dim3(MSM_THREADS), 0, st, buckets, parts, cap, t);
        }
    }

    int reduce() {
        static_assert(kKnobs[KNOB_PYR_TAIL_THREADS].dflt == PYR_TAIL_THREADS && kKnobs[KNOB_PYR_TAIL_BLOCKS].dflt == PYR_TAIL_BLOCKS, "knobs.hpp");
        const uint32_t tail_threads = (uint32_t)knob_int(KNOB_PYR_TAIL_THREADS), tail_blocks = (uint32_t)knob_int(KNOB_PYR_TAIL_BLOCKS);
        const uint32_t tail_half = (uint32_t)knob_int(KNOB_PYR_TAIL_HALF);
        if (tail_threads < 64 || tail_threads > 512 || (tail_threads & 63) || !tail_blocks || tail_blocks > 256 || !tail_half)
            return fail(ZKP_E_ARG, "ZKP_PYR_TAIL_THREADS must be a multiple of 64 up to 512, ZKP_PYR_TAIL_BLOCKS 1..256, ZKP_PYR_TAIL_HALF >= 1");
        for (size_t w = 0; w < W; w++) __atomic_store_n(result_flags + w, MSM_FLAG_PENDING, __ATOMIC_RELEASE);
        uint4* pyr[2] = {cx.buckets.get(), cx.pyr1.get()};
        uint4* odd[2] = {cx.odd0.get(), cx.odd1.get()};
        ProfScope ps("msm_bucket_reduce", st, true);
        uint32_t level_tail = 0;
        while (level_tail + 1 < g.c && (g.nb >> (level_tail + 1)) > tail_half) level_tail++;
        const uint32_t max_waves = cx.tail_max_waves;
        if ((uint64_t)g.nwin * (tail_threads / 64) > max_waves) level_tail = g.c - 1;
        for (uint32_t l = 0; l < level_tail; l++) {
            const PyrLevel L{l, g.nb >> (l + 1), g.nb, g.nwin};
            const bool quad = (uint64_t)L.half * (l + 1) * g.nwin <= (1u << 16);
            const uint32_t per = quad ? MSM_THREADS / 4 : MSM_THREADS;
            hipLaunchKernelGGL(quad ? msm_pyramid_quad_kernel : msm_pyramid_kernel, dim3((L.half + per - 1) / per, l + 1, g.nwin),
                               dim3(MSM_THREADS), 0, st, pyr[l & 1], pyr[(l + 1) & 1], odd[l & 1], odd[(l + 1) & 1], L);
        }
        if (level_tail + 1 < g.c) {
            uint32_t tb = tail_blocks;
            while (tb > 1 && (uint64_t)tb * g.nwin * (tail_threads / 64) > max_waves) tb >>= 1;
            const bool starve = knob_flag(KNOB_TEST_TAIL_STARVE);
            hipLaunchKernelGGL(msm_pyramid_tail_kernel, dim3(tb, g.nwin), dim3(tail_threads), 0, st, pyr[0], pyr[1], odd[0], odd[1], level_tail,
                               g.c, g.nb, cx.result.get(), result_out, result_flags, starve ? tb + 1 : tb, starve ? (1u << 12) : PYR_TAIL_SPIN_LIMIT);
        } else {
            const uint32_t fin = (g.c - 1) & 1;
            hipLaunchKernelGGL(msm_collect_kernel, dim3(g.nwin), dim3(64), 0, st, pyr[fin], pyr[fin ^ 1], odd[fin], g.nb, g.c, result_out,
                               result_flags);
        }
        return ZKP_OK;
    }
};

int wait_msm_result(const MsmGeom& g, const uint32_t* flags, hipStream_t st) {
    ZCHK(poll_or_sync(g.n <= (1ull << 24) && !knob_flag(KNOB_MSM_NO_POLL), st, [&] {
        for (size_t w = 0; w < g.nwin; w++)
            if (__atomic_load_n(flags + w, __ATOMIC_ACQUIRE) & MSM_FLAG_PENDING) return false;
        return true;
    }));
    for (size_t w = 0; w < g.nwin; w++)
        if (flags[w] & MSM_TAIL_TIMEOUT)
            return fail(ZKP_E_DEVICE, "bucket reduction: the workgroups of the last levels did not all become resident (device shared "
                                      "with another job?); no result was produced");
    return ZKP_OK;
}

HXyzz glv_phi(HXyzz v) {
    static const HFq beta = HFq::load(GlvParams::BETA).to_mont();
    v.x = v.x * beta;
    return v;
}
void msm_host_tail(const uint32_t* host_res, size_t count, uint32_t wins_per_msm, uint32_t c, bool glv, HXyzz* out) {
    const auto t_tail0 = std::chrono::steady_clock::now();
    auto tail_set = [&](size_t m) {
        const uint32_t* res = host_res + m * wins_per_msm * c * 64;
        HXyzz total = HXyzz::infinity();
        for (int pos = (int)(wins_per_msm * c) - 1; pos >= 0; pos--) {
            total = total.dbl();
            const int w = pos / (int)c, l = pos % (int)c;
            const uint32_t* rw = res + (size_t)w * c * 64;
            if (l <= (int)c - 2) total = total.add(xyzz_from_internal(rw + (size_t)(1 + l) * 64));
            if (l == 0) total = total.add(xyzz_from_internal(rw));
        }
        return total;
    };
    auto tail = [&](size_t m) { out[m] = glv ? tail_set(2 * m).add(glv_phi(tail_set(2 * m + 1))) : tail_set(m); };
    if (count == 1)
        tail(0);
    else
        host_pool().run(std::function<void(size_t)>(tail), count);
    prof_host("msm_tail_host", std::chrono::duration<double, std::milli>(std::chrono::steady_clock::now() - t_tail0).count());
}

int msm_partial_batch(const zkp_bases* bases, const Fr* const* d_scalars, size_t count, size_t n, hipStream_t st, HXyzz* out,
                      const MsmFeed* feed = nullptr) {
    MsmPlan p;
    if (const int rc = plan_msm({bases->n, bases->pre_c, bases->pre_planes, bases->pre_off, bases->pre_glv}, count, n, feed ? &feed->ranges : nullptr, &p))
        return fail(rc, p.error);
    if (p.lens.empty()) {
        for (size_t m = 0; m < count; m++) out[m] = HXyzz::infinity();
        return ZKP_OK;
    }
    MsmPass pass{p, p.g, bases, d_scalars, count, feed, st, st};
    ZCHK(pass.grow());
#ifdef ZKP_MSM_CHECK
    pass.dump(n);
#endif
    const int walk_rc = pass.walk(), up_rc = pass.up.join();
    if (walk_rc != ZKP_OK || up_rc != ZKP_OK) {
        if (p.overlap) (void)hipStreamSynchronize(pass.sst);
        if (feed) (void)hipStreamSynchronize(feed->copy_stream);
        return walk_rc != ZKP_OK ? walk_rc : fail(ZKP_E_DEVICE, "upload of a scalar range failed");
    }
    HIPCHK(hipGetLastError());
    ZCHK(pass.reduce());
    HIPCHK(hipGetLastError());
#ifdef ZKP_MSM_CHECK
    {
        uint32_t chk[32];
        HIPCHK(hipStreamSynchronize(st));
        HIPCHK(hipMemcpyFromSymbol(chk, HIP_SYMBOL(g_msm_check), sizeof(chk)));
        for (int k = 0; k < 8; k++)
            if (chk[4 * k]) fprintf(stderr, "ZKP_MSM_CHECK class %d: %u violations, first (%u, %u)\n", k, chk[4 * k], chk[4 * k + 1], chk[4 * k + 2]);
    }
#endif
    if (count > 1 && !knob_flag(KNOB_POOL_NO_WARM)) host_pool().warm(std::chrono::microseconds(3000));
    ZCHK(wait_msm_result(pass.g, pass.result_flags, st));
    msm_host_tail(reinterpret_cast<const uint32_t*>(pass.result_out), count, p.g.shared ? 1u : p.nwin1, p.g.c, p.g.glv != 0, out);
    return ZKP_OK;
}

int msm_partial(const zkp_bases* bases, const Fr* d_scalars, size_t n, hipStream_t st, HXyzz* out) {
    return msm_partial_batch(bases, &d_scalars, 1, n, st, out);
}
```

zkp-implementation_amd/csrc/plonk_host.inc:

```

struct PlonkScratch {
    Fr* ev;
    Fr* scan;
    uint64_t scan_cap;
    Fr* partial;
    unsigned partial_cap;
    uint64_t* h_pin;
    unsigned long long* poll_seq;
};

struct zkp_plonk_prover {
    const zkp_bases* srs = nullptr;
    unsigned log_n = 0, log_D = 0;
    uint64_t n = 0, D = 0, cap = 0;
    HFr k1, k2;
    int device = 0;
    TypedBuf<Fr> circ;
    TypedBuf<Fr> work;
    TypedBuf<Fr> t;
    TypedBuf<Fr> ev;
    TypedBuf<Fr> ev_w;
    Stream side;
    Event ev_fork, ev_abc, ev_z;
    TypedBuf<Fr> scan;
    uint64_t scan_cap = 0;
    TypedBuf<Fr> partial;
    unsigned partial_cap = 0;
    TypedBuf<unsigned long long> d_len;
    TypedBuf<Fr> dom_evals;
    uint64_t gates = 0;
    int gate_rows_bad = -1;
    bool perm_closes = false;
    TypedBuf<uint64_t, PinnedBuf> h_pin;
    unsigned long long poll_seq = 0;
    uint64_t t_len = 0, chunk = 0, r_len = 0, wz_len = 0, wzw_len = 0;
    int stage = 0;
    HFr beta, gamma, alpha, zeta, bar[6], pi_e;
    std::vector<HXyzz> para_table;
    bool fixed_evals_ready = false;
    bool consts_ready = false;
    HFr zh_inv[8], n_inv;
    PlonkScratch scratch() { return {ev, scan, scan_cap, partial, partial_cap, h_pin, &poll_seq}; }
    Fr* poly(int i) const { return work + (uint64_t)i * cap; }
    Fr* circuit(int i) const { return circ + (uint64_t)i * n; }
};

namespace {

enum { P_AX = 0, P_BX, P_CX, P_Z, P_R, P_WZ, P_WZW, P_TXC };
enum { C_QM = 0, C_QL, C_QR, C_QO, C_QC, C_PI, C_FA, C_FB, C_FC, C_S1, C_S2, C_S3 };

Fr fr_dev(const HFr& x) { Fr r; std::memcpy(r.l, x.l, 32); return r; }

__global__ void fr_add_at_kernel(Fr* d, uint64_t idx, Fr v) { d[idx] = d[idx] + v; }

int poke_add(Fr* d, uint64_t idx, const HFr& v, hipStream_t st) {
    hipLaunchKernelGGL(fr_add_at_kernel, dim3(1), dim3(1), 0, st, d, idx, fr_dev(v));
    HIPCHK(hipGetLastError());
    return ZKP_OK;
}

int blind_polys(zkp_plonk_prover* p, int count, Fr* const* dst, const Fr* const* src, const HFr (*c)[3], int len, hipStream_t st) {
    BlindParams bp;
    std::memset(&bp, 0, sizeof bp);
    for (int w = 0; w < count; w++) {
        bp.dst[w] = dst[w];
        bp.src[w] = src[w];
        for (int i = 0; i < len; i++) bp.c[w][i] = fr_dev(c[w][i]);
    }
    bp.len = (uint32_t)len;
    bp.n = p->n;
    bp.cap = p->cap;
    hipLaunchKernelGGL(plonk_blind_kernel, dim3((unsigned)((p->cap + PK_THREADS - 1) / PK_THREADS), (unsigned)count), dim3(PK_THREADS), 0, st, bp);
    HIPCHK(hipGetLastError());
    return ZKP_OK;
}

int commit_dev(const zkp_plonk_prover* p, const Fr* coeffs, uint64_t len, hipStream_t st, uint64_t out_xy[12], uint8_t* out_inf) {
    if (len > p->srs->n) return fail(ZKP_E_SIZE, "SRS shorter than the polynomial (kzg/src/scheme.rs:86)");
    HXyzz r;
    ZCHK(msm_partial(p->srs, coeffs, (size_t)len, st, &r));
    r.to_affine(out_xy, out_inf);
    return ZKP_OK;
}

int commit_batch_dev(const zkp_plonk_prover* p, const Fr* const* coeffs, size_t count, uint64_t len, hipStream_t st,
                     uint64_t* out_xy, uint8_t* out_inf) {
    if (len > p->srs->n) return fail(ZKP_E_SIZE, "SRS shorter than the polynomial (kzg/src/scheme.rs:86)");
    HXyzz r[8];
    if (count > 8) return fail(ZKP_E_ARG, "internal: batch too large");
    ZCHK(msm_partial_batch(p->srs, coeffs, count, (size_t)len, st, r));
    batch_to_affine(r, count, out_xy, out_inf);
    return ZKP_OK;
}

template <class Op>
int run_scan_batch(const PlonkScratch& s, const ScanJob* jobs, int count, hipStream_t st) {
    if (count < 1 || count > SCAN_MAX_BATCH) return fail(ZKP_E_ARG, "internal: scan batch");
    ScanParams sp;
    std::memset(&sp, 0, sizeof sp);
    uint64_t nmax = 0;
    for (int j = 0; j < count; j++) {
        sp.job[j] = jobs[j];
        nmax = std::max<uint64_t>(nmax, jobs[j].n);
    }
    if (nmax == 0) return ZKP_OK;
    sp.chunk = scan_chunk_for(nmax);
    const uint64_t blocks = scan_blocks_for(nmax);
    if (blocks > (1u << 20) || SCAN_MAX_BATCH * blocks * 257 > s.scan_cap) return fail(ZKP_E_ARG, "internal: scan scratch too small");
    sp.blocks = (uint32_t)blocks;
    sp.tpre = s.scan;
    sp.btot = s.scan + SCAN_MAX_BATCH * blocks * 256;
    const dim3 grid((unsigned)blocks, (unsigned)count);
    hipLaunchKernelGGL((scan_block_kernel<Op>), grid, dim3(256), 0, st, sp);
    hipLaunchKernelGGL((scan_mid_kernel<Op>), dim3(1, (unsigned)count), dim3(256), 0, st, sp);
    hipLaunchKernelGGL((scan_apply_kernel<Op>), grid, dim3(256), 0, st, sp);
    HIPCHK(hipGetLastError());
    return ZKP_OK;
}

struct EvalReq { const Fr* c; uint64_t len; HFr z; HFr* out; };
int wait_stream(const PlonkScratch& s, hipStream_t st) {
    if (!s.h_pin || knob_flag(KNOB_PLONK_NO_POLL)) {
        HIPCHK(hipStreamSynchronize(st));
        return ZKP_OK;
    }
    unsigned long long* flag = reinterpret_cast<unsigned long long*>(s.h_pin + 4 * (size_t)s.partial_cap);
    const unsigned long long seq = ++*s.poll_seq;
    hipLaunchKernelGGL(stream_signal_kernel, dim3(1), dim3(1), 0, st, flag, seq);
    HIPCHK(hipGetLastError());
    return poll_or_sync(true, st, [=] { return __atomic_load_n(flag, __ATOMIC_ACQUIRE) == seq; });
}

int eval_many_dev(const PlonkScratch& s, const std::vector<EvalReq>& reqs, hipStream_t st) {
    if (reqs.size() > EVAL_MAX_REQ) return fail(ZKP_E_ARG, "internal: too many evaluation requests");
    EvalParams ep;
    std::memset(&ep, 0, sizeof ep);
    std::vector<unsigned> blocks(reqs.size());
    std::vector<HFr> zblock(reqs.size());
    unsigned total = 0, max_blocks = 0;
    for (size_t i = 0; i < reqs.size(); i++) {
        const uint64_t threads = (reqs[i].len + EVAL_CHUNK - 1) / EVAL_CHUNK;
        blocks[i] = (unsigned)((threads + PK_THREADS - 1) / PK_THREADS);
        ep.c[i] = reqs[i].c;
        ep.len[i] = reqs[i].len;
        ep.part_off[i] = total;
        ep.z[i] = fr_dev(reqs[i].z);
        HFr zk = reqs[i].z.pow_u64(EVAL_CHUNK);
        for (int k = 0; k < 8; k++) {
            ep.zp[i][k] = fr_dev(zk);
            zk = zk * zk;
        }
        zblock[i] = zk;
        total += blocks[i];
        max_blocks = std::max(max_blocks, blocks[i]);
    }
    if (total > s.partial_cap) return fail(ZKP_E_ARG, "internal: evaluation scratch too small");
    if (max_blocks)
        hipLaunchKernelGGL(fr_poly_eval_kernel, dim3(max_blocks, (unsigned)reqs.size()), dim3(PK_THREADS), 0, st, ep, s.partial);
    HIPCHK(hipGetLastError());
    std::vector<uint64_t> pageable;
    uint64_t* h = s.h_pin;
    if (!h) {
        pageable.resize(4 * (size_t)std::max(total, 1u));
        h = pageable.data();
    }
    if (total) HIPCHK(hipMemcpyAsync(h, s.partial, 32 * (size_t)total, hipMemcpyDeviceToHost, st));
    ZCHK(wait_stream(s, st));
    for (size_t i = 0; i < reqs.size(); i++) {
        HFr acc = HFr::zero();
        for (unsigned b = blocks[i]; b-- > 0;) acc = acc * zblock[i] + HFr::load(&h[4 * (size_t)(ep.part_off[i] + b)]);
        *reqs[i].out = acc;
    }
    return ZKP_OK;
}
int eval_dev(const PlonkScratch& s, const Fr* c, uint64_t len, const HFr& z, hipStream_t st, HFr* out) {
    return eval_many_dev(s, {EvalReq{c, len, z, out}}, st);
}

int trim_len_dev(zkp_plonk_prover* p, const Fr* c, uint64_t n, hipStream_t st, uint64_t* len) {
    HIPCHK(hipMemsetAsync(p->d_len, 0, 8, st));
    hipLaunchKernelGGL(fr_trim_len_kernel, dim3((unsigned)((n + PK_THREADS - 1) / PK_THREADS)), dim3(PK_THREADS), 0, st, c, n,
                       p->d_len);
    HIPCHK(hipMemcpyAsync(p->h_pin, p->d_len, 8, hipMemcpyDeviceToHost, st));
    ZCHK(wait_stream(p->scratch(), st));
    *len = p->h_pin[0];
    return ZKP_OK;
}

ScalePowParams scale_pow_params(const HFr& base, uint64_t e0, uint32_t chunk) {
    ScalePowParams sp;
    sp.base = fr_dev(base);
    sp.c0 = fr_dev(base.pow_u64(e0));
    HFr b = base.pow_u64(chunk);
    for (int k = 0; k < 30; k++) {
        sp.bp[k] = fr_dev(b);
        b = b * b;
    }
    return sp;
}

struct DivReq { const Fr* c; uint64_t len; HFr z; Fr* out; };
int div_linear_batch_dev(const PlonkScratch& s, const DivReq* reqs, int count, hipStream_t st) {
    DivReq rq[2];
    int m = 0;
    for (int i = 0; i < count; i++) {
        if (reqs[i].len <= 1) continue;
        if (reqs[i].z.is_zero()) {
            HIPCHK(hipMemcpyAsync(reqs[i].out, reqs[i].c + 1, 32 * (reqs[i].len - 1), hipMemcpyDeviceToDevice, st));
            continue;
        }
        if (m == 2) return fail(ZKP_E_ARG, "internal: more than two divisions");
        rq[m++] = reqs[i];
    }
    if (!m) return ZKP_OK;
    uint64_t nmax = 0;
    for (int i = 0; i < m; i++) nmax = std::max(nmax, rq[i].len);
    const uint32_t chunk = (uint32_t)std::min<uint64_t>(8, std::max<uint64_t>(1, nmax >> 16));
    HFr zinv[2];
    if (m == 2) {
        const HFr pi = (rq[0].z * rq[1].z).inverse();
        zinv[0] = pi * rq[1].z;
        zinv[1] = pi * rq[0].z;
    } else {
        zinv[0] = rq[0].z.inverse();
    }
    ScalePowBatch fwd, back;
    std::memset(&fwd, 0, sizeof fwd);
    std::memset(&back, 0, sizeof back);
    ScanJob sj[2];
    Fr* scratch = s.ev;
    for (int i = 0; i < m; i++) {
        Fr* d = scratch;
        Fr* sfx = scratch + rq[i].len;
        scratch += 2 * rq[i].len;
        fwd.job[i] = ScalePowJob{rq[i].c, d, rq[i].len};
        fwd.sp[i] = scale_pow_params(rq[i].z, 0, chunk);
        sj[i] = ScanJob{d, sfx, rq[i].len, 1u, 1u};
        back.job[i] = ScalePowJob{sfx, rq[i].out, rq[i].len - 1};
        back.sp[i] = scale_pow_params(zinv[i], 1, chunk);
    }
    fwd.chunk = back.chunk = chunk;
    const dim3 grid((unsigned)(((nmax + chunk - 1) / chunk + PK_THREADS - 1) / PK_THREADS), (unsigned)m);
    hipLaunchKernelGGL(fr_scale_pow_kernel, grid, dim3(PK_THREADS), 0, st, fwd);
    ZCHK(run_scan_batch<OpAdd>(s, sj, m, st));
    hipLaunchKernelGGL(fr_scale_pow_kernel, grid, dim3(PK_THREADS), 0, st, back);
    HIPCHK(hipGetLastError());
    return ZKP_OK;
}
int div_linear_dev(const PlonkScratch& s, const Fr* c, uint64_t len, const HFr& z, Fr* out, hipStream_t st) {
    const DivReq r{c, len, z, out};
    return div_linear_batch_dev(s, &r, 1, st);
}

struct LcTerm { const Fr* p; uint64_t len; HFr s; };
int lincomb_dev(const std::vector<LcTerm>& terms, Fr* out, uint64_t n_out, hipStream_t st) {
    LincombParams L;
    std::memset(&L, 0, sizeof L);
    if (terms.size() > LINCOMB_MAX) return fail(ZKP_E_ARG, "too many terms");
    L.terms = (int)terms.size();
    L.n_out = n_out;
    for (size_t k = 0; k < terms.size(); k++) {
        L.p[k] = terms[k].p;
        L.len[k] = terms[k].len;
        L.s[k] = fr_dev(terms[k].s);
    }
    hipLaunchKernelGGL(fr_lincomb_kernel, dim3((unsigned)((n_out + PK_THREADS - 1) / PK_THREADS)), dim3(PK_THREADS), 0, st, L, out);
    HIPCHK(hipGetLastError());
    return ZKP_OK;
}

__global__ void fr_fill_kernel(Fr* p, uint64_t n, Fr v) {
    uint64_t i = (uint64_t)blockIdx.x * blockDim.x + threadIdx.x;
    if (i < n) p[i] = v;
}

const char* const kShardedSrsMsg = "SRS is sharded over several devices: a 2^16-gate proof does not shard (SURVEY 8e: replicas only) -- "
                                   "create the SRS on one slot (zkp_set_device) and run one prover per device";

int prover_alloc(const zkp_bases* srs, unsigned log_n, const HFr& k1, const HFr& k2, std::unique_ptr<zkp_plonk_prover>& p) {
    const uint64_t n = 1ull << log_n;
    if (srs->n < n + 3) return fail(ZKP_E_SIZE, "SRS must hold circuit_size + 3 points (kzg/src/srs.rs:51)");
    p.reset(new (std::nothrow) zkp_plonk_prover());
    if (!p) return fail(ZKP_E_NOMEM, "host allocation failed");
    p->srs = srs;
    p->device = ctx().device;
    p->log_n = log_n;
    p->n = n;
    p->log_D = log_n + 2;
    while ((1ull << p->log_D) < 3 * n + 7) p->log_D++;
    p->D = 1ull << p->log_D;
    p->cap = n + 8;
    p->k1 = k1;
    p->k2 = k2;
    HIPCHK_BARE(p->circ.grow(32 * 12 * n));
    HIPCHK_BARE(p->work.grow(32 * 8 * p->cap));
    HIPCHK_BARE(p->t.grow(32 * std::max<uint64_t>(p->D, 2 * p->cap)));
    HIPCHK_BARE(p->ev.grow(32 * 15 * p->D));
    HIPCHK_BARE(p->ev_w.grow(32 * 4 * p->D));
    HIPCHK_BARE(p->side.make(hipStreamNonBlocking));
    for (Event* ev : {&p->ev_fork, &p->ev_abc, &p->ev_z}) HIPCHK_BARE(ev->make(hipEventDisableTiming));
    p->scan_cap = scan_scratch_elems(p->D);
    HIPCHK_BARE(p->scan.grow(32 * p->scan_cap));
    p->partial_cap = (unsigned)(8 * (p->D / (EVAL_CHUNK * PK_THREADS) + 2));
    HIPCHK_BARE(p->partial.grow(32 * (size_t)p->partial_cap));
    HIPCHK_BARE(p->d_len.grow(8));
    HIPCHK_BARE(p->h_pin.grow(32 * (size_t)p->partial_cap + 128, hipHostMallocPortable | hipHostMallocMapped));
    p->h_pin[4 * (size_t)p->partial_cap] = 0;
    HIPCHK_BARE(hipMemset(p->circ, 0, 32 * 12 * n));
    HIPCHK_BARE(hipMemset(p->work, 0, 32 * 8 * p->cap));
    return ZKP_OK;
}

}

extern "C" {

int zkp_plonk_prover_create(const zkp_bases* srs, unsigned log_n, const uint64_t* const polys[12], const size_t lens[12],
                            const uint64_t k1[4], const uint64_t k2[4], zkp_plonk_prover** out) try {
    if (!srs || !polys || !lens || !k1 || !k2 || !out) return fail(ZKP_E_ARG, "null argument");
    if (log_n > 24) return fail(ZKP_E_ARG, "log_n > 24");
    if (!srs->shards.empty()) return fail(ZKP_E_ARG, kShardedSrsMsg);
    CTX_ENTER(srs->slot);
    WsOrder ord(nullptr);
    std::unique_ptr<zkp_plonk_prover> p;
    ZCHK(prover_alloc(srs, log_n, HFr::load(k1), HFr::load(k2), p));
    const uint64_t n = p->n;
    for (int i = 0; i < 12; i++) {
        if (lens[i] > n) return fail(ZKP_E_ARG, "circuit polynomial longer than n");
        if (lens[i]) HIPCHK_BARE(hipMemcpy(p->circuit(i), polys[i], 32 * lens[i], hipMemcpyHostToDevice));
    }
    *out = p.release();
    return ZKP_OK;
} ZKP_CATCH_INT

void zkp_plonk_prover_destroy(zkp_plonk_prover* p) {
    if (!p) return;
    if (p->side) (void)hipStreamSynchronize(p->side);
    DeviceRestore restore;
    (void)hipSetDevice(p->device);
    delete p;
}

static void prover_constants(zkp_plonk_prover* p) {
    if (p->consts_ready) return;
    const HFr g = HFr::from_u64(7);
    const uint32_t shift = (uint32_t)(p->D / p->n);
    HFr gn = g.pow_u64(p->n), ws = fr_root_of_unity(p->log_D - p->log_n), cur = HFr::one();
    HFr zh[8], prefix[8], run = HFr::one();
    for (uint32_t j = 0; j < 8 && j < shift; j++) {
        zh[j] = gn * cur - HFr::one();
        prefix[j] = run;
        run = run * zh[j];
        cur = cur * ws;
    }
    HFr inv = run.inverse();
    for (uint32_t j = 8; j-- > 0;) {
        if (j >= shift) { p->zh_inv[j] = HFr::zero(); continue; }
        p->zh_inv[j] = inv * prefix[j];
        inv = inv * zh[j];
    }
    HFr ninv = HFr::one(), half = HFr::from_u64(2).inverse();
    for (unsigned i = 0; i < p->log_n; i++) ninv = ninv * half;
    p->n_inv = ninv;
    p->consts_ready = true;
}

int witness_coset_async(zkp_plonk_prover* p, int first, int count, const Fr* const* src, const uint64_t* lens, hipStream_t st, hipEvent_t done) {
    const HFr g = HFr::from_u64(7);
    const uint64_t D = p->D;
    HIPCHK(hipEventRecord(p->ev_fork, st));
    HIPCHK(hipStreamWaitEvent(p->side, p->ev_fork, 0));
    HIPCHK(hipMemsetAsync(p->ev_w + (uint64_t)first * D, 0, 32 * (uint64_t)count * D, p->side));
    for (int i = 0; i < count; i++)
        HIPCHK(hipMemcpyAsync(p->ev_w + (uint64_t)(first + i) * D, src[i], 32 * lens[i], hipMemcpyDeviceToDevice, p->side));
    ZCHK(run_ntt<Fr>(p->ev_w + (uint64_t)first * D, p->log_D, (size_t)count, 0, g.l, p->side));
    HIPCHK(hipEventRecord(done, p->side));
    return ZKP_OK;
}

int zkp_plonk_round1(zkp_plonk_prover* p, const uint64_t* blinders , uint64_t* out_xy ,
                     uint8_t* out_inf ) try {
    if (!p || !blinders || !out_xy || !out_inf) return fail(ZKP_E_ARG, "null argument");
    CTX_ENTER(p->srs->slot);
    hipStream_t st = nullptr;
    WsOrder ord(st);
    const uint64_t n = p->n;
    {
        Fr* dst[3] = {p->poly(P_AX), p->poly(P_BX), p->poly(P_CX)};
        const Fr* src[3] = {p->circuit(C_FA), p->circuit(C_FB), p->circuit(C_FC)};
        HFr pre[3][3];
        for (int w = 0; w < 3; w++) {
            pre[w][0] = HFr::load(blinders + 4 * (2 * w + 1));
            pre[w][1] = HFr::load(blinders + 4 * (2 * w));
        }
        ZCHK(blind_polys(p, 3, dst, src, pre, 2, st));
    }
    const Fr* polys3[3] = {p->poly(P_AX), p->poly(P_BX), p->poly(P_CX)};
    {
        const uint64_t lens[3] = {n + 2, n + 2, n + 2};
        ZCHK(witness_coset_async(p, 0, 3, polys3, lens, st, p->ev_abc));
    }
    const int rc = commit_batch_dev(p, polys3, 3, n + 2, st, out_xy, out_inf);
    HIPCHK(hipEventSynchronize(p->ev_abc));
    ZCHK(rc);
    p->stage = 1;
    return ZKP_OK;
} ZKP_CATCH_INT

int zkp_plonk_round2(zkp_plonk_prover* p, const uint64_t beta[4], const uint64_t gamma[4], const uint64_t* blinders ,
                     uint64_t out_xy[12], uint8_t* out_inf) try {
    if (!p || !beta || !gamma || !blinders || !out_xy || !out_inf) return fail(ZKP_E_ARG, "null argument");
    if (p->stage < 1) return fail(ZKP_E_ARG, "round 1 has not run");
    CTX_ENTER(p->srs->slot);
    hipStream_t st = nullptr;
    WsOrder ord(st);
    const uint64_t n = p->n;
    p->beta = HFr::load(beta);
    p->gamma = HFr::load(gamma);
    if (!p->dom_evals) {
        TypedBuf<Fr> de_new;
        ZCHK(de_new.ensure(32 * 12 * n));
        int rc = ZKP_OK;
        if (hipMemcpyAsync(de_new, p->circ, 32 * 12 * n, hipMemcpyDeviceToDevice, st) != hipSuccess)
            rc = fail(ZKP_E_DEVICE, "copy of the circuit polynomials failed");
        if (rc == ZKP_OK) rc = run_ntt<Fr>(de_new, p->log_n, 12, 0, nullptr, st);
        if (rc == ZKP_OK) {
            if (hipMemsetAsync(p->d_len, 0, 8, st) != hipSuccess) rc = fail(ZKP_E_DEVICE, "memset failed");
            hipLaunchKernelGGL(plonk_gate_check_kernel, dim3((unsigned)((n + PK_THREADS - 1) / PK_THREADS)), dim3(PK_THREADS), 0, st,
                               de_new, n, p->d_len);
            if (rc == ZKP_OK && hipGetLastError() != hipSuccess) rc = fail(ZKP_E_DEVICE, "gate check launch failed");
            if (rc == ZKP_OK && hipMemcpyAsync(p->h_pin + 16, p->d_len, 8, hipMemcpyDeviceToHost, st) != hipSuccess)
                rc = fail(ZKP_E_DEVICE, "read-back failed");
        }
        if (rc == ZKP_OK && hipStreamSynchronize(st) != hipSuccess) rc = fail(ZKP_E_DEVICE, "gate check: synchronisation failed");
        if (rc != ZKP_OK) {
            (void)hipStreamSynchronize(st);
            return rc;
        }
        p->gate_rows_bad = (int)std::min<uint64_t>(p->h_pin[16], 1u << 30);
        p->dom_evals = std::move(de_new);
    }
    const Fr* de = p->dom_evals + 6 * n;
    AccParams ap;
    ap.a = de; ap.b = de + n; ap.c = de + 2 * n; ap.s1 = de + 3 * n; ap.s2 = de + 4 * n; ap.s3 = de + 5 * n;
    ap.beta = fr_dev(p->beta); ap.gamma = fr_dev(p->gamma); ap.k1 = fr_dev(p->k1); ap.k2 = fr_dev(p->k2);
    {
        HFr wk = fr_root_of_unity(p->log_n);
        for (int k = 0; k < 32; k++) {
            ap.wp[k] = fr_dev(wk);
            wk = wk.sqr();
        }
    }
    ap.n = n;
    Fr* num = p->ev + 6 * n;
    Fr* den = p->ev + 7 * n;
    Fr* nprefix = p->ev + 8 * n;
    Fr* dsuffix = p->ev + 9 * n;
    Fr* acc = p->ev + 10 * n;
    const unsigned nblocks = (unsigned)((n + PK_THREADS - 1) / PK_THREADS);
    hipLaunchKernelGGL(plonk_acc_numden_kernel, dim3(nblocks), dim3(PK_THREADS), 0, st, ap, num, den);
    HIPCHK(hipGetLastError());
    {
        const ScanJob sj[2] = {{num, nprefix, n, 0u, 1u}, {den, dsuffix, n, 1u, 0u}};
        ZCHK(run_scan_batch<OpMul>(p->scratch(), sj, 2, st));
    }
    uint64_t* total = p->h_pin;
    hipLaunchKernelGGL(fr_gather3_kernel, dim3(1), dim3(64), 0, st, dsuffix, nprefix + (n - 1), num + (n - 1), total);
    HIPCHK(hipGetLastError());
    ZCHK(wait_stream(p->scratch(), st));
    p->perm_closes = HFr::load(total + 4) * HFr::load(total + 8) == HFr::load(total);
    if (HFr::load(total) == HFr::zero())
        return fail(ZKP_E_ARG, "a permutation denominator is zero for these beta, gamma (rows 0 .. n-2: the reference divides by zero, "
                               "prover.rs:316,367; row n-1: the single-inversion accumulator of this prover cannot be formed)");
    const HFr inv_total = HFr::load(total).inverse();
    hipLaunchKernelGGL(plonk_acc_combine_kernel, dim3(nblocks), dim3(PK_THREADS), 0, st, nprefix, dsuffix, fr_dev(inv_total), n, acc);
    HIPCHK(hipGetLastError());
    ZCHK(run_ntt<Fr>(acc, p->log_n, 1, 1, nullptr, st));
    Fr* z = p->poly(P_Z);
    {
        Fr* dst[1] = {z};
        const Fr* src[1] = {acc};
        const HFr pre[1][3] = {{HFr::load(blinders + 8), HFr::load(blinders + 4), HFr::load(blinders)}};
        ZCHK(blind_polys(p, 1, dst, src, pre, 3, st));
    }
    {
        const Fr* zsrc[1] = {z};
        const uint64_t lens[1] = {n + 3};
        ZCHK(witness_coset_async(p, 3, 1, zsrc, lens, st, p->ev_z));
    }
    const int rc = commit_dev(p, z, n + 3, st, out_xy, out_inf);
    HIPCHK(hipEventSynchronize(p->ev_z));
    ZCHK(rc);
    p->stage = 2;
    return ZKP_OK;
} ZKP_CATCH_INT

int zkp_plonk_round3(zkp_plonk_prover* p, const uint64_t alpha[4], uint64_t* out_xy , uint8_t* out_inf ,
                     size_t* out_degree) try {
    if (!p || !alpha || !out_xy || !out_inf || !out_degree) return fail(ZKP_E_ARG, "null argument");
    if (p->stage < 2) return fail(ZKP_E_ARG, "round 2 has not run");
    CTX_ENTER(p->srs->slot);
    hipStream_t st = nullptr;
    WsOrder ord(st);
    const uint64_t n = p->n, D = p->D;
    p->alpha = HFr::load(alpha);
    const HFr g = HFr::from_u64(7);
    const int first_fixed = 4;
    if (!p->fixed_evals_ready) {
        HIPCHK(hipMemsetAsync(p->ev + (uint64_t)first_fixed * D, 0, 32 * (uint64_t)(15 - first_fixed) * D, st));
        const Fr* src[9] = {p->circuit(C_QM), p->circuit(C_QL), p->circuit(C_QR), p->circuit(C_QO), p->circuit(C_QC), p->circuit(C_PI),
                            p->circuit(C_S1), p->circuit(C_S2), p->circuit(C_S3)};
        for (int i = 0; i < 9; i++)
            HIPCHK(hipMemcpyAsync(p->ev + (uint64_t)(first_fixed + i) * D, src[i], 32 * n, hipMemcpyDeviceToDevice, st));
        prover_constants(p);
        const HFr ninv = p->n_inv;
        hipLaunchKernelGGL(fr_fill_kernel, dim3((unsigned)((n + 255) / 256)), dim3(256), 0, st, p->ev + 13 * D, n, fr_dev(ninv));
        uint64_t one[4];
        HFr::one().store(one);
        HIPCHK(hipMemcpyAsync(p->ev + 14 * D + 1, one, 32, hipMemcpyHostToDevice, st));
        ZCHK(run_ntt<Fr>(p->ev + (uint64_t)first_fixed * D, p->log_D, (size_t)(15 - first_fixed), 0, g.l, st));
    }
    p->fixed_evals_ready = true;
    QuotParams qp;
    qp.ev = p->ev;
    qp.w = p->ev_w;
    qp.D = D;
    qp.shift = (uint32_t)(D / n);
    qp.beta = fr_dev(p->beta); qp.gamma = fr_dev(p->gamma); qp.alpha = fr_dev(p->alpha); qp.alpha2 = fr_dev(p->alpha.sqr());
    qp.k1 = fr_dev(p->k1); qp.k2 = fr_dev(p->k2);
    if (qp.shift > 8) return fail(ZKP_E_ARG, "unsupported domain ratio");
    prover_constants(p);
    for (uint32_t j = 0; j < 8; j++) qp.zh_inv[j] = fr_dev(p->zh_inv[j]);
    hipLaunchKernelGGL(plonk_quotient_kernel, dim3((unsigned)((D + PK_THREADS - 1) / PK_THREADS)), dim3(PK_THREADS), 0, st, qp, p->t);
    HIPCHK(hipGetLastError());
    ZCHK(run_ntt<Fr>(p->t, p->log_D, 1, 1, g.l, st));
    ZCHK(trim_len_dev(p, p->t, D, st, &p->t_len));
    if (p->gate_rows_bad < 0) return fail(ZKP_E_DEVICE, "the gate rows of the witness were never checked (round 2 did not complete)");
    if (p->gate_rows_bad > 0)
        return fail(ZKP_E_ARG, "No remainder expected: " + std::to_string(p->gate_rows_bad) +
                                   " gate row(s) of the witness do not satisfy q_m ab + q_l a + q_r b + q_o c + pi + q_c = 0 (prover.rs:404)");
    if (!p->perm_closes)
        return fail(ZKP_E_ARG, "No remainder expected: the copy constraints do not hold, the permutation accumulator does not return to 1 (prover.rs:431)");
    if (p->t_len > 3 * n + 6) return fail(ZKP_E_ARG, "No remainder expected: circuit not satisfied (prover.rs:404,431,441)");
    if (p->t_len == 0) return fail(ZKP_E_ARG, "zero quotient polynomial cannot be sliced (slice_polynomial.rs:30)");
    p->chunk = (p->t_len + 2) / 3;
    {
        const Fr* sl[3] = {p->t, p->t + p->chunk, p->t + 2 * p->chunk};
        if (3 * p->chunk > std::max<uint64_t>(p->D, 2 * p->cap)) return fail(ZKP_E_ARG, "internal: slice overruns the buffer");
        ZCHK(commit_batch_dev(p, sl, 3, p->chunk, st, out_xy, out_inf));
    }
    *out_degree = (size_t)(p->chunk - 1);
    p->stage = 3;
    return ZKP_OK;
} ZKP_CATCH_INT

int zkp_plonk_round4(zkp_plonk_prover* p, const uint64_t zeta[4], uint64_t* out_bars ) try {
    if (!p || !zeta || !out_bars) return fail(ZKP_E_ARG, "null argument");
    if (p->stage < 3) return fail(ZKP_E_ARG, "round 3 has not run");
    CTX_ENTER(p->srs->slot);
    hipStream_t st = nullptr;
    WsOrder ord(st);
    const uint64_t n = p->n;
    p->zeta = HFr::load(zeta);
    const HFr w = fr_root_of_unity(p->log_n);
    ZCHK(eval_many_dev(p->scratch(), {{p->poly(P_AX), n + 2, p->zeta, &p->bar[0]}, {p->poly(P_BX), n + 2, p->zeta, &p->bar[1]},
                           {p->poly(P_CX), n + 2, p->zeta, &p->bar[2]}, {p->circuit(C_S1), n, p->zeta, &p->bar[3]},
                           {p->circuit(C_S2), n, p->zeta, &p->bar[4]}, {p->poly(P_Z), n + 3, p->zeta * w, &p->bar[5]},
                           {p->circuit(C_PI), n, p->zeta, &p->pi_e}}, st));
    std::vector<LcTerm> terms;
    HFr zc = p->zeta.pow_u64(p->chunk), cur = HFr::one();
    for (int i = 0; i < 3; i++) {
        const uint64_t off = (uint64_t)i * p->chunk;
        const uint64_t len = off < p->t_len ? std::min<uint64_t>(p->chunk, p->t_len - off) : 0;
        terms.push_back(LcTerm{p->t + off, len, cur});
        cur = cur * zc;
    }
    ZCHK(lincomb_dev(terms, p->poly(P_TXC), p->chunk, st));
    for (int i = 0; i < 6; i++) p->bar[i].store(out_bars + 4 * i);
    p->stage = 4;
    return ZKP_OK;
} ZKP_CATCH_INT

int zkp_plonk_round5(zkp_plonk_prover* p, const uint64_t v_limbs[4], uint64_t* out_xy , uint8_t* out_inf ) try {
    if (!p || !v_limbs || !out_xy || !out_inf) return fail(ZKP_E_ARG, "null argument");
    if (p->stage < 4) return fail(ZKP_E_ARG, "round 4 has not run");
    CTX_ENTER(p->srs->slot);
    hipStream_t st = nullptr;
    WsOrder ord(st);
    const uint64_t n = p->n;
    const HFr v = HFr::load(v_limbs);
    const HFr &beta = p->beta, &gamma = p->gamma, &alpha = p->alpha, &zeta = p->zeta;
    const HFr &ba = p->bar[0], &bb = p->bar[1], &bc = p->bar[2], &bs1 = p->bar[3], &bs2 = p->bar[4], &bzw = p->bar[5];
    const HFr w = fr_root_of_unity(p->log_n);
    const HFr c2 = (ba + beta * zeta + gamma) * (bb + beta * p->k1 * zeta + gamma) * (bc + beta * p->k2 * zeta + gamma) * alpha;
    const HFr c3 = (ba + beta * bs1 + gamma) * (bb + beta * bs2 + gamma) * bzw * alpha;
    const HFr zn = zeta.pow_u64(n);
    const HFr zh = zn - HFr::one();
    prover_constants(p);
    const HFr ninv = p->n_inv;
    HFr l1e;
    if (zeta == HFr::one()) l1e = HFr::one();
    else l1e = ninv * zh * (zeta - HFr::one()).inverse();
    const HFr c4 = l1e * alpha.sqr();
    std::vector<LcTerm> terms = {
        {p->circuit(C_QM), n, ba * bb}, {p->circuit(C_QL), n, ba}, {p->circuit(C_QR), n, bb}, {p->circuit(C_QO), n, bc},
        {p->circuit(C_QC), n, HFr::one()}, {p->poly(P_Z), n + 3, c2 + c4}, {p->circuit(C_S3), n, (beta * c3).neg()},
        {p->poly(P_TXC), p->chunk, zh.neg()}};
    p->r_len = std::max<uint64_t>(n + 3, p->chunk);
    if (p->r_len > p->cap) return fail(ZKP_E_ARG, "internal: linearisation longer than the working capacity");
    Fr* r = p->poly(P_R);
    ZCHK(lincomb_dev(terms, r, p->r_len, st));
    ZCHK(poke_add(r, 0, p->pi_e - (bc + gamma) * c3 - c4, st));
    HFr bar_r;
    ZCHK(eval_dev(p->scratch(), r, p->r_len, zeta, st, &bar_r));
    const HFr v2 = v * v, v3 = v2 * v, v4 = v3 * v, v5 = v4 * v;
    std::vector<LcTerm> wt = {{r, p->r_len, HFr::one()}, {p->poly(P_AX), n + 2, v}, {p->poly(P_BX), n + 2, v2},
                              {p->poly(P_CX), n + 2, v3}, {p->circuit(C_S1), n, v4}, {p->circuit(C_S2), n, v5}};
    Fr* num = p->t;
    ZCHK(lincomb_dev(wt, num, p->r_len, st));
    ZCHK(poke_add(num, 0, (bar_r + v * ba + v2 * bb + v3 * bc + v4 * bs1 + v5 * bs2).neg(), st));
    p->wz_len = p->r_len - 1;
    Fr* num2 = p->t + p->cap;
    HIPCHK(hipMemcpyAsync(num2, p->poly(P_Z), 32 * (n + 3), hipMemcpyDeviceToDevice, st));
    ZCHK(poke_add(num2, 0, bzw.neg(), st));
    {
        const DivReq dv[2] = {{num, p->r_len, zeta, p->poly(P_WZ)}, {num2, n + 3, zeta * w, p->poly(P_WZW)}};
        ZCHK(div_linear_batch_dev(p->scratch(), dv, 2, st));
    }
    p->wzw_len = n + 2;
    if (p->wz_len == p->wzw_len) {
        const Fr* ws[2] = {p->poly(P_WZ), p->poly(P_WZW)};
        ZCHK(commit_batch_dev(p, ws, 2, p->wz_len, st, out_xy, out_inf));
    } else {
        ZCHK(commit_dev(p, p->poly(P_WZ), p->wz_len, st, out_xy, out_inf));
        ZCHK(commit_dev(p, p->poly(P_WZW), p->wzw_len, st, out_xy + 12, out_inf + 1));
    }
    p->stage = 5;
    return ZKP_OK;
} ZKP_CATCH_INT

int zkp_plonk_get_poly(zkp_plonk_prover* p, int which, uint64_t* out, size_t cap_elems, size_t* len) try {
    if (!p || !len) return fail(ZKP_E_ARG, "null argument");
    CTX_ENTER(p->srs->slot);
    WsOrder ord(nullptr);
    const Fr* src = nullptr;
    uint64_t l = 0;
    const uint64_t n = p->n;
    switch (which) {
        case 0: case 1: case 2: src = p->poly(which); l = n + 2; break;
        case 3: src = p->poly(P_Z); l = n + 3; break;
        case 4: src = p->poly(P_R); l = p->r_len; break;
        case 5: src = p->poly(P_WZ); l = p->wz_len; break;
        case 6: src = p->poly(P_WZW); l = p->wzw_len; break;
        case 7: src = p->poly(P_TXC); l = p->chunk; break;
        case 8: src = p->t; l = p->stage >= 5 ? 0 : p->t_len; break;
        default: return fail(ZKP_E_ARG, "unknown polynomial id");
    }
    *len = (size_t)l;
    const size_t m = std::min<size_t>(cap_elems, (size_t)l);
    if (m && out) HIPCHK(hipMemcpy(out, src, 32 * m, hipMemcpyDeviceToHost));
    return ZKP_OK;
} ZKP_CATCH_INT

}

uint64_t open_scratch_elems(uint64_t len) {
    return 3 * len + scan_scratch_elems(len) + len / (EVAL_CHUNK * PK_THREADS) + 2;
}

int open_eval_div_dev(Fr* scratch, const Fr* d_c, uint64_t len, const HFr& z, hipStream_t st, HFr* y, Fr** q_out) {
    const uint64_t n_tot = scan_scratch_elems(len);
    Fr* d_q = scratch;
    Fr* ev = d_q + len;
    const PlonkScratch w{ev, ev + 2 * len, n_tot, ev + 2 * len + n_tot, (unsigned)(len / (EVAL_CHUNK * PK_THREADS) + 2), nullptr, nullptr};
    ZCHK(eval_dev(w, d_c, len, z, st, y));
    if (len > 1) ZCHK(div_linear_dev(w, d_c, len, z, d_q, st));
    *q_out = d_q;
    return ZKP_OK;
}

int kzg_open_device(const zkp_bases* srs, const uint64_t* coeffs, size_t len, const uint64_t z_limbs[4], uint64_t out_xy[12],
                    uint8_t* out_is_inf, uint64_t out_eval[4]) {
    len = trimmed_len(coeffs, len);
    if (len == 0) {
        std::memset(out_eval, 0, 32);
        std::memset(out_xy, 0, 96);
        *out_is_inf = 1;
        return ZKP_OK;
    }
    if (len - 1 > srs->n) return fail(ZKP_E_SIZE, "SRS shorter than the quotient polynomial (kzg/src/scheme.rs:86)");
    const bool sharded = !srs->shards.empty();
    std::vector<uint64_t> h_q;
    HXyzz r = HXyzz::infinity();
    {
        CTX_ENTER(sharded ? srs->shards[0]->slot : srs->slot);
        hipStream_t st = nullptr;
        WsOrder ord(st);
        ZCHK(ctx().tmp.ensure(32 * (len + open_scratch_elems(len)) + 64));
        Fr* d_c = reinterpret_cast<Fr*>(ctx().tmp.p);
        HIPCHK(hipMemcpyAsync(d_c, coeffs, 32 * len, hipMemcpyHostToDevice, st));
        HFr y;
        Fr* d_q = nullptr;
        ZCHK(open_eval_div_dev(d_c + len, d_c, len, HFr::load(z_limbs), st, &y, &d_q));
        y.store(out_eval);
        if (len > 1) {
            if (sharded) {
                h_q.resize(4 * (len - 1));
                HIPCHK(hipMemcpyAsync(h_q.data(), d_q, 32 * (len - 1), hipMemcpyDeviceToHost, st));
                HIPCHK(hipStreamSynchronize(st));
            } else {
                ZCHK(msm_partial(srs, d_q, len - 1, st, &r));
            }
        }
    }
    if (sharded && len > 1) ZCHK(msm_host_scalars_any(srs, h_q.data(), len - 1, &r));
    r.to_affine(out_xy, out_is_inf);
    return ZKP_OK;
}

namespace {

int build_para_table(zkp_plonk_prover* p) {
    uint32_t raw[32];
    {
        CTX_ENTER(p->srs->slot);
        WsOrder ord(nullptr);
        if (!p->srs->n) return fail(ZKP_E_SIZE, "empty SRS (unwrap() at kzg/src/scheme.rs:79)");
        HIPCHK(hipMemcpy(raw, p->srs->d_xy.p, 128, hipMemcpyDeviceToHost));
    }
    HXyzz base{fq_from_limbs28(raw), fq_from_limbs28(raw + 16), HFq::one(), HFq::one()};
    p->para_table.resize(64 * 15);
    for (int w = 0; w < 64; w++) {
        HXyzz cur = base;
        for (int d = 0; d < 15; d++) {
            p->para_table[w * 15 + d] = cur;
            cur = cur.add(base);
        }
        for (int k = 0; k < 4; k++) base = base.dbl();
    }
    const size_t cnt = p->para_table.size();
    std::vector<uint64_t> xy(12 * cnt);
    std::vector<uint8_t> inf(cnt);
    batch_to_affine(p->para_table.data(), cnt, xy.data(), inf.data());
    for (size_t i = 0; i < cnt; i++) p->para_table[i] = HXyzz::from_affine(&xy[12 * i], false);
    return ZKP_OK;
}

HXyzz commit_para_xyzz(const zkp_plonk_prover* p, const HFr& para) {
    const HFr k = para.from_mont();
    HXyzz acc = HXyzz::infinity();
    for (int w = 0; w < 64; w++) {
        const unsigned d = (unsigned)(k.l[w >> 4] >> (4 * (w & 15))) & 15u;
        if (d) acc = acc.madd(p->para_table[w * 15 + d - 1].x, p->para_table[w * 15 + d - 1].y);
    }
    return acc;
}

void commit_para(const zkp_plonk_prover* p, const HFr& para, uint64_t out_xy[12], uint8_t* out_inf) {
    commit_para_xyzz(p, para).to_affine(out_xy, out_inf);
}

}

extern "C" int zkp_plonk_prove(zkp_plonk_prover* p, const uint64_t* blinders , zkp_plonk_proof* out) try {
    if (!p || !blinders || !out) return fail(ZKP_E_ARG, "null argument");
    if (p->srs->d_inf.p) return fail(ZKP_E_ARG, "SRS with infinity points");
    if (p->para_table.empty()) ZCHK(build_para_table(p));
    std::memset(out, 0, sizeof *out);
    PlonkChallengeGenerator ch;
    auto feed = [&](int i) {
        uint64_t x[6] = {0}, y[6] = {0};
        if (!out->commit_is_inf[i]) {
            const HFq cx = HFq::load(out->commit_xy[i]).from_mont(), cy = HFq::load(out->commit_xy[i] + 6).from_mont();
            std::memcpy(x, cx.l, 48);
            std::memcpy(y, cy.l, 48);
        }
        ch.feed(x, y, out->commit_is_inf[i] != 0);
    };
    uint64_t c2[8], c1[4];
    ZCHK(zkp_plonk_round1(p, blinders, out->commit_xy[0], out->commit_is_inf));
    feed(0); feed(1); feed(2);
    ch.generate(2, c2);
    ZCHK(zkp_plonk_round2(p, c2, c2 + 4, blinders + 24, out->commit_xy[3], out->commit_is_inf + 3));
    feed(3);
    ch.generate(1, c1);
    size_t degree = 0;
    ZCHK(zkp_plonk_round3(p, c1, out->commit_xy[4], out->commit_is_inf + 4, &degree));
    out->degree = degree;
    feed(4); feed(5); feed(6);
    ch.generate(1, c1);
    ZCHK(zkp_plonk_round4(p, c1, out->bars[0]));
    HXyzz para[6];
    uint64_t para_xy[6 * 12];
    uint8_t para_inf[6];
    {
        const std::function<void(size_t)> job = [&](size_t i) { para[i] = commit_para_xyzz(p, HFr::load(out->bars[i])); };
        host_pool().run(job, 6);
    }
    batch_to_affine(para, 6, para_xy, para_inf);
    for (int i = 0; i < 6; i++) {
        const uint64_t* xy = para_xy + 12 * i;
        const uint8_t inf = para_inf[i];
        uint64_t x[6] = {0}, y[6] = {0};
        if (!inf) {
            const HFq cx = HFq::load(xy).from_mont(), cy = HFq::load(xy + 6).from_mont();
            std::memcpy(x, cx.l, 48);
            std::memcpy(y, cy.l, 48);
        }
        ch.feed(x, y, inf != 0);
    }
    ch.generate(1, c1);
    ZCHK(zkp_plonk_round5(p, c1, out->commit_xy[7], out->commit_is_inf + 7));
    feed(7); feed(8);
    ch.generate(1, out->u);
    return ZKP_OK;
} ZKP_CATCH_INT
```

Measured before the change: 442.4 million.

## Overlap PLONK linearisation eval, precompute division constants, spin-wait host pool, add host profiling

Moves the linearisation polynomial build and its evaluation launch from round 5 into round 4 so the evaluation runs on the device while the host computes the para commitments. Division constants are precomputed, and repeated evaluation points reuse their z powers. The host pool spin-waits briefly before blocking on the condition variable. The prove path calls the round bodies directly, and per-phase host timing laps are added. The G1 MSM path itself only gains timing marks and a refactored tail, so the MSM metric is unlikely to move.

Measured after the change: 441.3 million. About the same (-0.3%).

```diff
diff --git a/zkp-implementation_amd/build.py b/zkp-implementation_amd/build.py
--- a/zkp-implementation_amd/build.py
+++ b/zkp-implementation_amd/build.py
@@ -8,7 +8,7 @@
 OUT = os.path.join(HERE, "libzkp_hip.so")
 SOURCES = ["api.hip", "selftest.hip"]
 DEPS = ["api.hip", "ff.hpp", "fq28.hpp", "fq28_inv.hpp", "fr29.hpp", "fr29_mul2_asm.inc", "fq28_mul_asm.inc", "fq28_mul2x_asm.inc", "fq28_sqr_asm.inc", "fq28_mul2_asm.inc", "g1.hpp", "g1_28.hpp", "msm.hpp", "ntt.hpp", "ntt_plan.hpp", "ntt_host.inc", "plonk.hpp",
-        "plonk_host.inc", "plonk_compile_host.inc", "ntt_sharded.inc", "fri.hpp", "fri_host.inc", "fri_fr.hpp", "transcript_host.hpp", "pairing_host.hpp", "verify_host.inc", "host_ff.hpp", "kzg_host.hpp", "host_threads.hpp", "knobs.hpp", "msm_plan.hpp", "glv.hpp", "g1_check.hpp", "g1_check_host.inc", "g1_ntt.hpp", "g1_ntt_plan.hpp", "g1_ntt_host.inc", "msm_host.inc", "nova.hpp", "nova_host.inc", "dev_res.hpp", "selftest.hpp", "selftest.hip",
+        "plonk_host.inc", "plonk_compile_host.inc", "ntt_sharded.inc", "fri.hpp", "fri_host.inc", "fri_fr.hpp", "transcript_host.hpp", "pairing_host.hpp", "verify_host.inc", "host_ff.hpp", "kzg_host.hpp", "host_threads.hpp", "knobs.hpp", "msm_plan.hpp", "glv.hpp", "g1_check.hpp", "g1_check_host.inc", "g1_ntt.hpp", "g1_ntt_plan.hpp", "g1_ntt_host.inc", "msm_host.inc", "msm_tail.hpp", "nova.hpp", "nova_host.inc", "dev_res.hpp", "selftest.hpp", "selftest.hip",
         os.path.join("..", "..", "include", "zkp_hip.h")]
 
 
diff --git a/zkp-implementation_amd/csrc/api.hip b/zkp-implementation_amd/csrc/api.hip
--- a/zkp-implementation_amd/csrc/api.hip
+++ b/zkp-implementation_amd/csrc/api.hip
@@ -84,6 +84,7 @@
     } while (0)
 
 #include "host_threads.hpp"
+#include "msm_tail.hpp"
 #include "dev_res.hpp"
 static_assert(ZKP_HOST_THREADS_E_DEVICE == ZKP_E_DEVICE && ZKP_HOST_THREADS_OK == ZKP_OK, "host_threads.hpp error codes");
 
@@ -194,6 +195,57 @@
     r.host_ms = ms;
     prof_records().push_back(std::move(r));
 }
+
+enum HostCat { H_LAUNCH = 0, H_PLAN, H_WAIT, H_TAIL, H_AFFINE, H_TRANSCRIPT, H_SCALARS, H_READBACK, H_PARA, H_ENTRY, H_CATS };
+#define ZKP_HOST_ROUNDS(c) {"plonk_host_" c ".r0", "plonk_host_" c ".r1", "plonk_host_" c ".r2", "plonk_host_" c ".r3", "plonk_host_" c ".r4", "plonk_host_" c ".r5"}
+static const char* const kHostPhase[H_CATS][6] = {ZKP_HOST_ROUNDS("launch"), ZKP_HOST_ROUNDS("plan"), ZKP_HOST_ROUNDS("wait"), ZKP_HOST_ROUNDS("tail"),
+                                                  ZKP_HOST_ROUNDS("affine"), ZKP_HOST_ROUNDS("transcript"), ZKP_HOST_ROUNDS("scalars"),
+                                                  ZKP_HOST_ROUNDS("readback"), ZKP_HOST_ROUNDS("para"), ZKP_HOST_ROUNDS("entry")};
+#undef ZKP_HOST_ROUNDS
+struct HostLap;
+thread_local HostLap* t_lap = nullptr;
+struct HostLap {
+    using clock = std::chrono::steady_clock;
+    const int round;
+    bool on;
+    HostLap* prev = nullptr;
+    clock::time_point last;
+    double ms[H_CATS] = {0};
+    bool used[H_CATS] = {false};
+    explicit HostLap(int r) : round(r), on(g_prof_on.load(std::memory_order_relaxed) == 1) {
+        if (!on) return;
+        prev = t_lap;
+        t_lap = this;
+        last = clock::now();
+    }
+    void mark(HostCat c) {
+        const clock::time_point now = clock::now();
+        ms[c] += std::chrono::duration<double, std::milli>(now - last).count();
+        used[c] = true;
+        last = now;
+    }
+    void flush() {
+        for (int c = 0; on && c < H_CATS; c++)
+            if (used[c]) prof_host(kHostPhase[c][round], ms[c]);
+        close();
+    }
+    void close() {
+        if (on) t_lap = prev;
+        on = false;
+    }
+    ~HostLap() { close(); }
+};
+inline void host_mark(HostCat c) { if (t_lap) t_lap->mark(c); }
+struct RoundLap : HostLap {
+    explicit RoundLap(int r) : HostLap(r) { if (on && prev) prev->mark(H_ENTRY); }
+    ~RoundLap() {
+        if (!on) return;
+        mark(H_ENTRY);
+        HostLap* outer = prev;
+        flush();
+        if (outer) outer->last = clock::now();
+    }
+};
 
 enum { CLK_MSM_ACCUMULATE = 0, CLK_MAD_PROBE = 1, CLK_NTT_FR = 2, CLK_NTT_GL = 3, CLK_COUNT = 4 };
 static const char* const kClkNames[CLK_COUNT] = {"msm_accumulate", "mad_probe", "ntt_fr_pass", "ntt_gl_pass"};
@@ -483,8 +535,9 @@
     for (const auto& c : g_rt.slots) {
         std::lock_guard<std::mutex> lk(c->mu);
         HIPCHK(hipSetDevice(c->device));
+        const size_t name_len = std::strlen(name);
         for (ProfRec& r : c->prof) {
-            if (std::strcmp(r.name, name) != 0) continue;
+            if (std::strcmp(r.name, name) != 0 && !(std::strncmp(r.name, name, name_len) == 0 && r.name[name_len] == '.')) continue;
             if (r.a) {
                 HIPCHK(hipEventSynchronize(r.b));
                 float ms = 0;
diff --git a/zkp-implementation_amd/csrc/host_threads.hpp b/zkp-implementation_amd/csrc/host_threads.hpp
--- a/zkp-implementation_amd/csrc/host_threads.hpp
+++ b/zkp-implementation_amd/csrc/host_threads.hpp
@@ -22,6 +22,7 @@
     size_t next = 0, total = 0, finished = 0;
     bool started = false;
     std::atomic<bool> posted{false};
+    std::atomic<size_t> finished_seen{0};
     std::chrono::steady_clock::time_point warm_until{};
     void worker() {
         std::unique_lock<std::mutex> lk(mu);
@@ -42,7 +43,8 @@
             lk.unlock();
             (*f)(i);
             lk.lock();
-            if (++finished == total) cv_done.notify_one();
+            finished_seen.store(++finished, std::memory_order_release);
+            if (finished == total) cv_done.notify_one();
         }
     }
 
@@ -58,6 +60,7 @@
         next = 0;
         total = n;
         finished = 0;
+        finished_seen.store(0, std::memory_order_relaxed);
         warm_until = {};
         posted.store(true, std::memory_order_release);
         cv.notify_all();
@@ -66,7 +69,14 @@
             lk.unlock();
             f(i);
             lk.lock();
-            ++finished;
+            finished_seen.store(++finished, std::memory_order_release);
+        }
+        if (finished != total) {
+            lk.unlock();
+            const auto until = std::chrono::steady_clock::now() + std::chrono::microseconds(200);
+            for (unsigned spins = 0; finished_seen.load(std::memory_order_acquire) != n; __builtin_ia32_pause())
+                if ((++spins & 63) == 0 && std::chrono::steady_clock::now() >= until) break;
+            lk.lock();
         }
         cv_done.wait(lk, [&] { return finished == total; });
         fn = nullptr;
diff --git a/zkp-implementation_amd/csrc/msm_host.inc b/zkp-implementation_amd/csrc/msm_host.inc
--- a/zkp-implementation_amd/csrc/msm_host.inc
+++ b/zkp-implementation_amd/csrc/msm_host.inc
@@ -248,30 +248,9 @@
     return ZKP_OK;
 }
 
-HXyzz glv_phi(HXyzz v) {
-    static const HFq beta = HFq::load(GlvParams::BETA).to_mont();
-    v.x = v.x * beta;
-    return v;
-}
 void msm_host_tail(const uint32_t* host_res, size_t count, uint32_t wins_per_msm, uint32_t c, bool glv, HXyzz* out) {
     const auto t_tail0 = std::chrono::steady_clock::now();
-    auto tail_set = [&](size_t m) {
-        const uint32_t* res = host_res + m * wins_per_msm * c * 64;
-        HXyzz total = HXyzz::infinity();
-        for (int pos = (int)(wins_per_msm * c) - 1; pos >= 0; pos--) {
-            total = total.dbl();
-            const int w = pos / (int)c, l = pos % (int)c;
-            const uint32_t* rw = res + (size_t)w * c * 64;
-            if (l <= (int)c - 2) total = total.add(xyzz_from_internal(rw + (size_t)(1 + l) * 64));
-            if (l == 0) total = total.add(xyzz_from_internal(rw));
-        }
-        return total;
-    };
-    auto tail = [&](size_t m) { out[m] = glv ? tail_set(2 * m).add(glv_phi(tail_set(2 * m + 1))) : tail_set(m); };
-    if (count == 1)
-        tail(0);
-    else
-        host_pool().run(std::function<void(size_t)>(tail), count);
+    msm_tail_fanout(host_pool(), host_res, count, wins_per_msm, c, glv, out);
     prof_host("msm_tail_host", std::chrono::duration<double, std::milli>(std::chrono::steady_clock::now() - t_tail0).count());
 }
 
@@ -286,6 +265,7 @@
     }
     MsmPass pass{p, p.g, bases, d_scalars, count, feed, st, st};
     ZCHK(pass.grow());
+    host_mark(H_PLAN);
 #ifdef ZKP_MSM_CHECK
     pass.dump(n);
 #endif
@@ -308,8 +288,11 @@
     }
 #endif
     if (count > 1 && !knob_flag(KNOB_POOL_NO_WARM)) host_pool().warm(std::chrono::microseconds(3000));
+    host_mark(H_LAUNCH);
     ZCHK(wait_msm_result(pass.g, pass.result_flags, st));
+    host_mark(H_WAIT);
     msm_host_tail(reinterpret_cast<const uint32_t*>(pass.result_out), count, p.g.shared ? 1u : p.nwin1, p.g.c, p.g.glv != 0, out);
+    host_mark(H_TAIL);
     return ZKP_OK;
 }
 
diff --git a/zkp-implementation_amd/csrc/msm_tail.hpp b/zkp-implementation_amd/csrc/msm_tail.hpp
--- /dev/null
+++ b/zkp-implementation_amd/csrc/msm_tail.hpp
@@ -0,0 +1,38 @@
+#pragma once
+
+inline HXyzz glv_phi(HXyzz v) {
+    static const HFq beta = HFq::load(GlvParams::BETA).to_mont();
+    v.x = v.x * beta;
+    return v;
+}
+
+inline HXyzz msm_tail_set(const uint32_t* res, uint32_t wins, uint32_t c) {
+    HXyzz total = HXyzz::infinity();
+    for (int pos = (int)(wins * c) - 1; pos >= 0; pos--) {
+        total = total.dbl();
+        const int w = pos / (int)c, l = pos % (int)c;
+        const uint32_t* rw = res + (size_t)w * c * 64;
+        if (l <= (int)c - 2) total = total.add(xyzz_from_internal(rw + (size_t)(1 + l) * 64));
+        if (l == 0) total = total.add(xyzz_from_internal(rw));
+    }
+    return total;
+}
+
+inline HXyzz msm_tail_one(const uint32_t* host_res, size_t m, uint32_t wins_per_msm, uint32_t c, bool glv) {
+    const size_t set_words = (size_t)wins_per_msm * c * 64;
+    if (!glv) return msm_tail_set(host_res + m * set_words, wins_per_msm, c);
+    return msm_tail_set(host_res + 2 * m * set_words, wins_per_msm, c).add(glv_phi(msm_tail_set(host_res + (2 * m + 1) * set_words, wins_per_msm, c)));
+}
+
+inline void msm_tail_serial(const uint32_t* host_res, size_t count, uint32_t wins_per_msm, uint32_t c, bool glv, HXyzz* out) {
+    for (size_t m = 0; m < count; m++) out[m] = msm_tail_one(host_res, m, wins_per_msm, c, glv);
+}
+
+inline void msm_tail_fanout(HostPool& pool, const uint32_t* host_res, size_t count, uint32_t wins_per_msm, uint32_t c, bool glv, HXyzz* out) {
+    if (count <= 1) {
+        msm_tail_serial(host_res, count, wins_per_msm, c, glv, out);
+        return;
+    }
+    const std::function<void(size_t)> job = [=](size_t m) { out[m] = msm_tail_one(host_res, m, wins_per_msm, c, glv); };
+    pool.run(job, count);
+}
diff --git a/zkp-implementation_amd/csrc/plonk_host.inc b/zkp-implementation_amd/csrc/plonk_host.inc
--- a/zkp-implementation_amd/csrc/plonk_host.inc
+++ b/zkp-implementation_amd/csrc/plonk_host.inc
@@ -7,6 +7,23 @@
     unsigned partial_cap;
     uint64_t* h_pin;
     unsigned long long* poll_seq;
+};
+
+struct StreamTicket { unsigned long long seq = 0; bool polled = false; };
+struct EvalPending {
+    bool active = false;
+    std::vector<unsigned> blocks, off;
+    std::vector<HFr> zblock;
+    std::vector<HFr*> out;
+    const uint64_t* h = nullptr;
+    StreamTicket ticket;
+};
+struct DivPre {
+    bool ready = false;
+    HFr z[2];
+    uint64_t len[2] = {0, 0};
+    uint32_t chunk = 0;
+    ScalePowParams fwd[2], back[2];
 };
 
 struct zkp_plonk_prover {
@@ -33,6 +50,13 @@
     bool perm_closes = false;
     TypedBuf<uint64_t, PinnedBuf> h_pin;
     unsigned long long poll_seq = 0;
+    TypedBuf<Fr> partial_r;
+    unsigned partial_r_cap = 0;
+    TypedBuf<uint64_t, PinnedBuf> h_pin_r;
+    unsigned long long poll_seq_r = 0;
+    EvalPending r_eval;
+    HFr bar_r;
+    DivPre div_pre;
     uint64_t t_len = 0, chunk = 0, r_len = 0, wz_len = 0, wzw_len = 0;
     int stage = 0;
     HFr beta, gamma, alpha, zeta, bar[6], pi_e;
@@ -41,6 +65,7 @@
     bool consts_ready = false;
     HFr zh_inv[8], n_inv;
     PlonkScratch scratch() { return {ev, scan, scan_cap, partial, partial_cap, h_pin, &poll_seq}; }
+    PlonkScratch scratch_r() { return {ev, scan, scan_cap, partial_r, partial_r_cap, h_pin_r, &poll_seq_r}; }
     Fr* poly(int i) const { return work + (uint64_t)i * cap; }
     Fr* circuit(int i) const { return circ + (uint64_t)i * n; }
 };
@@ -79,8 +104,10 @@
 int commit_dev(const zkp_plonk_prover* p, const Fr* coeffs, uint64_t len, hipStream_t st, uint64_t out_xy[12], uint8_t* out_inf) {
     if (len > p->srs->n) return fail(ZKP_E_SIZE, "SRS shorter than the polynomial (kzg/src/scheme.rs:86)");
     HXyzz r;
+    host_mark(H_LAUNCH);
     ZCHK(msm_partial(p->srs, coeffs, (size_t)len, st, &r));
     r.to_affine(out_xy, out_inf);
+    host_mark(H_AFFINE);
     return ZKP_OK;
 }
 
@@ -89,8 +116,10 @@
     if (len > p->srs->n) return fail(ZKP_E_SIZE, "SRS shorter than the polynomial (kzg/src/scheme.rs:86)");
     HXyzz r[8];
     if (count > 8) return fail(ZKP_E_ARG, "internal: batch too large");
+    host_mark(H_LAUNCH);
     ZCHK(msm_partial_batch(p->srs, coeffs, count, (size_t)len, st, r));
     batch_to_affine(r, count, out_xy, out_inf);
+    host_mark(H_AFFINE);
     return ZKP_OK;
 }
 
@@ -120,59 +149,105 @@
 }
 
 struct EvalReq { const Fr* c; uint64_t len; HFr z; HFr* out; };
+int signal_stream(const PlonkScratch& s, hipStream_t st, StreamTicket* t) {
+    host_mark(H_LAUNCH);
+    t->polled = s.h_pin && !knob_flag(KNOB_PLONK_NO_POLL);
+    if (!t->polled) return ZKP_OK;
+    unsigned long long* flag = reinterpret_cast<unsigned long long*>(s.h_pin + 4 * (size_t)s.partial_cap);
+    t->seq = ++*s.poll_seq;
+    hipLaunchKernelGGL(stream_signal_kernel, dim3(1), dim3(1), 0, st, flag, t->seq);
+    HIPCHK(hipGetLastError());
+    host_mark(H_LAUNCH);
+    return ZKP_OK;
+}
+int await_stream(const PlonkScratch& s, hipStream_t st, const StreamTicket& t) {
+    int rc = ZKP_OK;
+    if (!t.polled) {
+        const hipError_t e = hipStreamSynchronize(st);
+        if (e != hipSuccess) rc = hip_fail(e, "hipStreamSynchronize(st): ");
+    } else {
+        const unsigned long long* flag = reinterpret_cast<const unsigned long long*>(s.h_pin + 4 * (size_t)s.partial_cap);
+        const unsigned long long seq = t.seq;
+        rc = poll_or_sync(true, st, [=] { return __atomic_load_n(flag, __ATOMIC_ACQUIRE) == seq; });
+    }
+    host_mark(H_READBACK);
+    return rc;
+}
 int wait_stream(const PlonkScratch& s, hipStream_t st) {
-    if (!s.h_pin || knob_flag(KNOB_PLONK_NO_POLL)) {
-        HIPCHK(hipStreamSynchronize(st));
-        return ZKP_OK;
-    }
-    unsigned long long* flag = reinterpret_cast<unsigned long long*>(s.h_pin + 4 * (size_t)s.partial_cap);
-    const unsigned long long seq = ++*s.poll_seq;
-    hipLaunchKernelGGL(stream_signal_kernel, dim3(1), dim3(1), 0, st, flag, seq);
-    HIPCHK(hipGetLastError());
-    return poll_or_sync(true, st, [=] { return __atomic_load_n(flag, __ATOMIC_ACQUIRE) == seq; });
-}
-
-int eval_many_dev(const PlonkScratch& s, const std::vector<EvalReq>& reqs, hipStream_t st) {
+    StreamTicket t;
+    ZCHK(signal_stream(s, st, &t));
+    return await_stream(s, st, t);
+}
+
+int eval_many_launch(const PlonkScratch& s, const std::vector<EvalReq>& reqs, hipStream_t st, uint64_t* h, EvalPending* pend) {
     if (reqs.size() > EVAL_MAX_REQ) return fail(ZKP_E_ARG, "internal: too many evaluation requests");
     EvalParams ep;
     std::memset(&ep, 0, sizeof ep);
-    std::vector<unsigned> blocks(reqs.size());
-    std::vector<HFr> zblock(reqs.size());
+    pend->active = false;
+    pend->blocks.assign(reqs.size(), 0);
+    pend->off.assign(reqs.size(), 0);
+    pend->zblock.assign(reqs.size(), HFr::zero());
+    pend->out.assign(reqs.size(), nullptr);
     unsigned total = 0, max_blocks = 0;
     for (size_t i = 0; i < reqs.size(); i++) {
         const uint64_t threads = (reqs[i].len + EVAL_CHUNK - 1) / EVAL_CHUNK;
-        blocks[i] = (unsigned)((threads + PK_THREADS - 1) / PK_THREADS);
+        pend->blocks[i] = (unsigned)((threads + PK_THREADS - 1) / PK_THREADS);
+        pend->out[i] = reqs[i].out;
         ep.c[i] = reqs[i].c;
         ep.len[i] = reqs[i].len;
-        ep.part_off[i] = total;
+        ep.part_off[i] = pend->off[i] = total;
         ep.z[i] = fr_dev(reqs[i].z);
-        HFr zk = reqs[i].z.pow_u64(EVAL_CHUNK);
-        for (int k = 0; k < 8; k++) {
-            ep.zp[i][k] = fr_dev(zk);
-            zk = zk * zk;
+        size_t same = i;
+        for (size_t j = 0; j < i && same == i; j++)
+            if (reqs[j].z == reqs[i].z) same = j;
+        if (same != i) {
+            for (int k = 0; k < 8; k++) ep.zp[i][k] = ep.zp[same][k];
+            pend->zblock[i] = pend->zblock[same];
+        } else {
+            HFr zk = reqs[i].z.pow_u64(EVAL_CHUNK);
+            for (int k = 0; k < 8; k++) {
+                ep.zp[i][k] = fr_dev(zk);
+                zk = zk * zk;
+            }
+            pend->zblock[i] = zk;
         }
-        zblock[i] = zk;
-        total += blocks[i];
-        max_blocks = std::max(max_blocks, blocks[i]);
+        total += pend->blocks[i];
+        max_blocks = std::max(max_blocks, pend->blocks[i]);
     }
     if (total > s.partial_cap) return fail(ZKP_E_ARG, "internal: evaluation scratch too small");
+    host_mark(H_SCALARS);
     if (max_blocks)
         hipLaunchKernelGGL(fr_poly_eval_kernel, dim3(max_blocks, (unsigned)reqs.size()), dim3(PK_THREADS), 0, st, ep, s.partial);
     HIPCHK(hipGetLastError());
+    if (total) HIPCHK(hipMemcpyAsync(h, s.partial, 32 * (size_t)total, hipMemcpyDeviceToHost, st));
+    ZCHK(signal_stream(s, st, &pend->ticket));
+    pend->h = h;
+    pend->active = true;
+    return ZKP_OK;
+}
+int eval_many_finish(const PlonkScratch& s, EvalPending* pend, hipStream_t st) {
+    pend->active = false;
+    ZCHK(await_stream(s, st, pend->ticket));
+    for (size_t i = 0; i < pend->out.size(); i++) {
+        HFr acc = HFr::zero();
+        for (unsigned b = pend->blocks[i]; b-- > 0;) acc = acc * pend->zblock[i] + HFr::load(&pend->h[4 * (size_t)(pend->off[i] + b)]);
+        *pend->out[i] = acc;
+    }
+    host_mark(H_SCALARS);
+    return ZKP_OK;
+}
+int eval_many_dev(const PlonkScratch& s, const std::vector<EvalReq>& reqs, hipStream_t st) {
     std::vector<uint64_t> pageable;
     uint64_t* h = s.h_pin;
     if (!h) {
-        pageable.resize(4 * (size_t)std::max(total, 1u));
+        size_t total = 0;
+        for (const EvalReq& r : reqs) total += (size_t)(((r.len + EVAL_CHUNK - 1) / EVAL_CHUNK + PK_THREADS - 1) / PK_THREADS);
+        pageable.resize(4 * std::max<size_t>(total, 1));
         h = pageable.data();
     }
-    if (total) HIPCHK(hipMemcpyAsync(h, s.partial, 32 * (size_t)total, hipMemcpyDeviceToHost, st));
-    ZCHK(wait_stream(s, st));
-    for (size_t i = 0; i < reqs.size(); i++) {
-        HFr acc = HFr::zero();
-        for (unsigned b = blocks[i]; b-- > 0;) acc = acc * zblock[i] + HFr::load(&h[4 * (size_t)(ep.part_off[i] + b)]);
-        *reqs[i].out = acc;
-    }
-    return ZKP_OK;
+    EvalPending pend;
+    ZCHK(eval_many_launch(s, reqs, st, h, &pend));
+    return eval_many_finish(s, &pend, st);
 }
 int eval_dev(const PlonkScratch& s, const Fr* c, uint64_t len, const HFr& z, hipStream_t st, HFr* out) {
     return eval_many_dev(s, {EvalReq{c, len, z, out}}, st);
@@ -201,7 +276,20 @@
 }
 
 struct DivReq { const Fr* c; uint64_t len; HFr z; Fr* out; };
-int div_linear_batch_dev(const PlonkScratch& s, const DivReq* reqs, int count, hipStream_t st) {
+uint32_t div_chunk_for(uint64_t nmax) { return (uint32_t)std::min<uint64_t>(8, std::max<uint64_t>(1, nmax >> 16)); }
+void div_constants(const HFr z[2], const uint64_t len[2], DivPre* d) {
+    d->chunk = div_chunk_for(std::max(len[0], len[1]));
+    const HFr pi = (z[0] * z[1]).inverse();
+    const HFr zinv[2] = {pi * z[1], pi * z[0]};
+    for (int i = 0; i < 2; i++) {
+        d->z[i] = z[i];
+        d->len[i] = len[i];
+        d->fwd[i] = scale_pow_params(z[i], 0, d->chunk);
+        d->back[i] = scale_pow_params(zinv[i], 1, d->chunk);
+    }
+    d->ready = true;
+}
+int div_linear_batch_dev(const PlonkScratch& s, const DivReq* reqs, int count, hipStream_t st, const DivPre* pre = nullptr) {
     DivReq rq[2];
     int m = 0;
     for (int i = 0; i < count; i++) {
@@ -216,15 +304,16 @@
     if (!m) return ZKP_OK;
     uint64_t nmax = 0;
     for (int i = 0; i < m; i++) nmax = std::max(nmax, rq[i].len);
-    const uint32_t chunk = (uint32_t)std::min<uint64_t>(8, std::max<uint64_t>(1, nmax >> 16));
-    HFr zinv[2];
-    if (m == 2) {
-        const HFr pi = (rq[0].z * rq[1].z).inverse();
-        zinv[0] = pi * rq[1].z;
-        zinv[1] = pi * rq[0].z;
-    } else {
-        zinv[0] = rq[0].z.inverse();
-    }
+    const uint32_t chunk = div_chunk_for(nmax);
+    DivPre own;
+    if (m == 2 && !(pre && pre->ready && pre->z[0] == rq[0].z && pre->z[1] == rq[1].z && pre->len[0] == rq[0].len && pre->len[1] == rq[1].len)) {
+        const HFr z[2] = {rq[0].z, rq[1].z};
+        const uint64_t len[2] = {rq[0].len, rq[1].len};
+        div_constants(z, len, &own);
+        pre = &own;
+    }
+    HFr zinv0;
+    if (m == 1) zinv0 = rq[0].z.inverse();
     ScalePowBatch fwd, back;
     std::memset(&fwd, 0, sizeof fwd);
     std::memset(&back, 0, sizeof back);
@@ -235,12 +324,13 @@
         Fr* sfx = scratch + rq[i].len;
         scratch += 2 * rq[i].len;
         fwd.job[i] = ScalePowJob{rq[i].c, d, rq[i].len};
-        fwd.sp[i] = scale_pow_params(rq[i].z, 0, chunk);
+        fwd.sp[i] = m == 2 ? pre->fwd[i] : scale_pow_params(rq[i].z, 0, chunk);
         sj[i] = ScanJob{d, sfx, rq[i].len, 1u, 1u};
         back.job[i] = ScalePowJob{sfx, rq[i].out, rq[i].len - 1};
-        back.sp[i] = scale_pow_params(zinv[i], 1, chunk);
+        back.sp[i] = m == 2 ? pre->back[i] : scale_pow_params(zinv0, 1, chunk);
     }
     fwd.chunk = back.chunk = chunk;
+    host_mark(H_SCALARS);
     const dim3 grid((unsigned)(((nmax + chunk - 1) / chunk + PK_THREADS - 1) / PK_THREADS), (unsigned)m);
     hipLaunchKernelGGL(fr_scale_pow_kernel, grid, dim3(PK_THREADS), 0, st, fwd);
     ZCHK(run_scan_batch<OpAdd>(s, sj, m, st));
@@ -307,6 +397,10 @@
     HIPCHK_BARE(p->d_len.grow(8));
     HIPCHK_BARE(p->h_pin.grow(32 * (size_t)p->partial_cap + 128, hipHostMallocPortable | hipHostMallocMapped));
     p->h_pin[4 * (size_t)p->partial_cap] = 0;
+    p->partial_r_cap = (unsigned)(p->cap / (EVAL_CHUNK * PK_THREADS) + 2);
+    HIPCHK_BARE(p->partial_r.grow(32 * (size_t)p->partial_r_cap));
+    HIPCHK_BARE(p->h_pin_r.grow(32 * (size_t)p->partial_r_cap + 128, hipHostMallocPortable | hipHostMallocMapped));
+    p->h_pin_r[4 * (size_t)p->partial_r_cap] = 0;
     HIPCHK_BARE(hipMemset(p->circ, 0, 32 * 12 * n));
     HIPCHK_BARE(hipMemset(p->work, 0, 32 * 8 * p->cap));
     return ZKP_OK;
@@ -379,12 +473,9 @@
     return ZKP_OK;
 }
 
-int zkp_plonk_round1(zkp_plonk_prover* p, const uint64_t* blinders , uint64_t* out_xy ,
-                     uint8_t* out_inf ) try {
-    if (!p || !blinders || !out_xy || !out_inf) return fail(ZKP_E_ARG, "null argument");
-    CTX_ENTER(p->srs->slot);
-    hipStream_t st = nullptr;
-    WsOrder ord(st);
+static int round1_body(zkp_plonk_prover* p, const uint64_t* blinders , uint64_t* out_xy ,
+                     uint8_t* out_inf , hipStream_t st) {
+    RoundLap lap(1);
     const uint64_t n = p->n;
     {
         Fr* dst[3] = {p->poly(P_AX), p->poly(P_BX), p->poly(P_CX)};
@@ -403,18 +494,23 @@
     }
     const int rc = commit_batch_dev(p, polys3, 3, n + 2, st, out_xy, out_inf);
     HIPCHK(hipEventSynchronize(p->ev_abc));
+    host_mark(H_WAIT);
     ZCHK(rc);
     p->stage = 1;
     return ZKP_OK;
-} ZKP_CATCH_INT
-
-int zkp_plonk_round2(zkp_plonk_prover* p, const uint64_t beta[4], const uint64_t gamma[4], const uint64_t* blinders ,
-                     uint64_t out_xy[12], uint8_t* out_inf) try {
-    if (!p || !beta || !gamma || !blinders || !out_xy || !out_inf) return fail(ZKP_E_ARG, "null argument");
-    if (p->stage < 1) return fail(ZKP_E_ARG, "round 1 has not run");
+}
+int zkp_plonk_round1(zkp_plonk_prover* p, const uint64_t* blinders , uint64_t* out_xy ,
+                     uint8_t* out_inf ) try {
+    if (!p || !blinders || !out_xy || !out_inf) return fail(ZKP_E_ARG, "null argument");
     CTX_ENTER(p->srs->slot);
     hipStream_t st = nullptr;
     WsOrder ord(st);
+    return round1_body(p, blinders, out_xy, out_inf, st);
+} ZKP_CATCH_INT
+
+static int round2_body(zkp_plonk_prover* p, const uint64_t beta[4], const uint64_t gamma[4], const uint64_t* blinders ,
+                     uint64_t out_xy[12], uint8_t* out_inf, hipStream_t st) {
+    RoundLap lap(2);
     const uint64_t n = p->n;
     p->beta = HFr::load(beta);
     p->gamma = HFr::load(gamma);
@@ -459,6 +555,7 @@
     Fr* dsuffix = p->ev + 9 * n;
     Fr* acc = p->ev + 10 * n;
     const unsigned nblocks = (unsigned)((n + PK_THREADS - 1) / PK_THREADS);
+    host_mark(H_SCALARS);
     hipLaunchKernelGGL(plonk_acc_numden_kernel, dim3(nblocks), dim3(PK_THREADS), 0, st, ap, num, den);
     HIPCHK(hipGetLastError());
     {
@@ -474,6 +571,7 @@
         return fail(ZKP_E_ARG, "a permutation denominator is zero for these beta, gamma (rows 0 .. n-2: the reference divides by zero, "
                                "prover.rs:316,367; row n-1: the single-inversion accumulator of this prover cannot be formed)");
     const HFr inv_total = HFr::load(total).inverse();
+    host_mark(H_SCALARS);
     hipLaunchKernelGGL(plonk_acc_combine_kernel, dim3(nblocks), dim3(PK_THREADS), 0, st, nprefix, dsuffix, fr_dev(inv_total), n, acc);
     HIPCHK(hipGetLastError());
     ZCHK(run_ntt<Fr>(acc, p->log_n, 1, 1, nullptr, st));
@@ -491,18 +589,24 @@
     }
     const int rc = commit_dev(p, z, n + 3, st, out_xy, out_inf);
     HIPCHK(hipEventSynchronize(p->ev_z));
+    host_mark(H_WAIT);
     ZCHK(rc);
     p->stage = 2;
     return ZKP_OK;
-} ZKP_CATCH_INT
-
-int zkp_plonk_round3(zkp_plonk_prover* p, const uint64_t alpha[4], uint64_t* out_xy , uint8_t* out_inf ,
-                     size_t* out_degree) try {
-    if (!p || !alpha || !out_xy || !out_inf || !out_degree) return fail(ZKP_E_ARG, "null argument");
-    if (p->stage < 2) return fail(ZKP_E_ARG, "round 2 has not run");
+}
+int zkp_plonk_round2(zkp_plonk_prover* p, const uint64_t beta[4], const uint64_t gamma[4], const uint64_t* blinders ,
+                     uint64_t out_xy[12], uint8_t* out_inf) try {
+    if (!p || !beta || !gamma || !blinders || !out_xy || !out_inf) return fail(ZKP_E_ARG, "null argument");
+    if (p->stage < 1) return fail(ZKP_E_ARG, "round 1 has not run");
     CTX_ENTER(p->srs->slot);
     hipStream_t st = nullptr;
     WsOrder ord(st);
+    return round2_body(p, beta, gamma, blinders, out_xy, out_inf, st);
+} ZKP_CATCH_INT
+
+static int round3_body(zkp_plonk_prover* p, const uint64_t alpha[4], uint64_t* out_xy , uint8_t* out_inf ,
+                     size_t* out_degree, hipStream_t st) {
+    RoundLap lap(3);
     const uint64_t n = p->n, D = p->D;
     p->alpha = HFr::load(alpha);
     const HFr g = HFr::from_u64(7);
@@ -532,6 +636,7 @@
     if (qp.shift > 8) return fail(ZKP_E_ARG, "unsupported domain ratio");
     prover_constants(p);
     for (uint32_t j = 0; j < 8; j++) qp.zh_inv[j] = fr_dev(p->zh_inv[j]);
+    host_mark(H_SCALARS);
     hipLaunchKernelGGL(plonk_quotient_kernel, dim3((unsigned)((D + PK_THREADS - 1) / PK_THREADS)), dim3(PK_THREADS), 0, st, qp, p->t);
     HIPCHK(hipGetLastError());
     ZCHK(run_ntt<Fr>(p->t, p->log_D, 1, 1, g.l, st));
@@ -553,46 +658,21 @@
     *out_degree = (size_t)(p->chunk - 1);
     p->stage = 3;
     return ZKP_OK;
-} ZKP_CATCH_INT
-
-int zkp_plonk_round4(zkp_plonk_prover* p, const uint64_t zeta[4], uint64_t* out_bars ) try {
-    if (!p || !zeta || !out_bars) return fail(ZKP_E_ARG, "null argument");
-    if (p->stage < 3) return fail(ZKP_E_ARG, "round 3 has not run");
+}
+int zkp_plonk_round3(zkp_plonk_prover* p, const uint64_t alpha[4], uint64_t* out_xy , uint8_t* out_inf ,
+                     size_t* out_degree) try {
+    if (!p || !alpha || !out_xy || !out_inf || !out_degree) return fail(ZKP_E_ARG, "null argument");
+    if (p->stage < 2) return fail(ZKP_E_ARG, "round 2 has not run");
     CTX_ENTER(p->srs->slot);
     hipStream_t st = nullptr;
     WsOrder ord(st);
+    return round3_body(p, alpha, out_xy, out_inf, out_degree, st);
+} ZKP_CATCH_INT
+
+static int linearisation_async(zkp_plonk_prover* p, hipStream_t st) {
     const uint64_t n = p->n;
-    p->zeta = HFr::load(zeta);
-    const HFr w = fr_root_of_unity(p->log_n);
-    ZCHK(eval_many_dev(p->scratch(), {{p->poly(P_AX), n + 2, p->zeta, &p->bar[0]}, {p->poly(P_BX), n + 2, p->zeta, &p->bar[1]},
-                           {p->poly(P_CX), n + 2, p->zeta, &p->bar[2]}, {p->circuit(C_S1), n, p->zeta, &p->bar[3]},
-                           {p->circuit(C_S2), n, p->zeta, &p->bar[4]}, {p->poly(P_Z), n + 3, p->zeta * w, &p->bar[5]},
-                           {p->circuit(C_PI), n, p->zeta, &p->pi_e}}, st));
-    std::vector<LcTerm> terms;
-    HFr zc = p->zeta.pow_u64(p->chunk), cur = HFr::one();
-    for (int i = 0; i < 3; i++) {
-        const uint64_t off = (uint64_t)i * p->chunk;
-        const uint64_t len = off < p->t_len ? std::min<uint64_t>(p->chunk, p->t_len - off) : 0;
-        terms.push_back(LcTerm{p->t + off, len, cur});
-        cur = cur * zc;
-    }
-    ZCHK(lincomb_dev(terms, p->poly(P_TXC), p->chunk, st));
-    for (int i = 0; i < 6; i++) p->bar[i].store(out_bars + 4 * i);
-    p->stage = 4;
-    return ZKP_OK;
-} ZKP_CATCH_INT
-
-int zkp_plonk_round5(zkp_plonk_prover* p, const uint64_t v_limbs[4], uint64_t* out_xy , uint8_t* out_inf ) try {
-    if (!p || !v_limbs || !out_xy || !out_inf) return fail(ZKP_E_ARG, "null argument");
-    if (p->stage < 4) return fail(ZKP_E_ARG, "round 4 has not run");
-    CTX_ENTER(p->srs->slot);
-    hipStream_t st = nullptr;
-    WsOrder ord(st);
-    const uint64_t n = p->n;
-    const HFr v = HFr::load(v_limbs);
     const HFr &beta = p->beta, &gamma = p->gamma, &alpha = p->alpha, &zeta = p->zeta;
     const HFr &ba = p->bar[0], &bb = p->bar[1], &bc = p->bar[2], &bs1 = p->bar[3], &bs2 = p->bar[4], &bzw = p->bar[5];
-    const HFr w = fr_root_of_unity(p->log_n);
     const HFr c2 = (ba + beta * zeta + gamma) * (bb + beta * p->k1 * zeta + gamma) * (bc + beta * p->k2 * zeta + gamma) * alpha;
     const HFr c3 = (ba + beta * bs1 + gamma) * (bb + beta * bs2 + gamma) * bzw * alpha;
     const HFr zn = zeta.pow_u64(n);
@@ -610,13 +690,68 @@
     p->r_len = std::max<uint64_t>(n + 3, p->chunk);
     if (p->r_len > p->cap) return fail(ZKP_E_ARG, "internal: linearisation longer than the working capacity");
     Fr* r = p->poly(P_R);
+    host_mark(H_SCALARS);
     ZCHK(lincomb_dev(terms, r, p->r_len, st));
     ZCHK(poke_add(r, 0, p->pi_e - (bc + gamma) * c3 - c4, st));
-    HFr bar_r;
-    ZCHK(eval_dev(p->scratch(), r, p->r_len, zeta, st, &bar_r));
+    const std::vector<EvalReq> req = {EvalReq{r, p->r_len, zeta, &p->bar_r}};
+    ZCHK(eval_many_launch(p->scratch_r(), req, st, p->h_pin_r, &p->r_eval));
+    return ZKP_OK;
+}
+
+static int round4_body(zkp_plonk_prover* p, const uint64_t zeta[4], uint64_t* out_bars , hipStream_t st) {
+    RoundLap lap(4);
+    const uint64_t n = p->n;
+    p->zeta = HFr::load(zeta);
+    const HFr w = fr_root_of_unity(p->log_n);
+    ZCHK(eval_many_dev(p->scratch(), {{p->poly(P_AX), n + 2, p->zeta, &p->bar[0]}, {p->poly(P_BX), n + 2, p->zeta, &p->bar[1]},
+                           {p->poly(P_CX), n + 2, p->zeta, &p->bar[2]}, {p->circuit(C_S1), n, p->zeta, &p->bar[3]},
+                           {p->circuit(C_S2), n, p->zeta, &p->bar[4]}, {p->poly(P_Z), n + 3, p->zeta * w, &p->bar[5]},
+                           {p->circuit(C_PI), n, p->zeta, &p->pi_e}}, st));
+    std::vector<LcTerm> terms;
+    HFr zc = p->zeta.pow_u64(p->chunk), cur = HFr::one();
+    for (int i = 0; i < 3; i++) {
+        const uint64_t off = (uint64_t)i * p->chunk;
+        const uint64_t len = off < p->t_len ? std::min<uint64_t>(p->chunk, p->t_len - off) : 0;
+        terms.push_back(LcTerm{p->t + off, len, cur});
+        cur = cur * zc;
+    }
+    host_mark(H_SCALARS);
+    ZCHK(lincomb_dev(terms, p->poly(P_TXC), p->chunk, st));
+    for (int i = 0; i < 6; i++) p->bar[i].store(out_bars + 4 * i);
+    ZCHK(linearisation_async(p, st));
+    {
+        const HFr z[2] = {p->zeta, p->zeta * w};
+        const uint64_t len[2] = {p->r_len, n + 3};
+        p->div_pre.ready = false;
+        if (!z[0].is_zero() && !z[1].is_zero() && len[0] > 1 && len[1] > 1) div_constants(z, len, &p->div_pre);
+    }
+    host_mark(H_SCALARS);
+    p->stage = 4;
+    return ZKP_OK;
+}
+int zkp_plonk_round4(zkp_plonk_prover* p, const uint64_t zeta[4], uint64_t* out_bars ) try {
+    if (!p || !zeta || !out_bars) return fail(ZKP_E_ARG, "null argument");
+    if (p->stage < 3) return fail(ZKP_E_ARG, "round 3 has not run");
+    CTX_ENTER(p->srs->slot);
+    hipStream_t st = nullptr;
+    WsOrder ord(st);
+    return round4_body(p, zeta, out_bars, st);
+} ZKP_CATCH_INT
+
+static int round5_body(zkp_plonk_prover* p, const uint64_t v_limbs[4], uint64_t* out_xy , uint8_t* out_inf , hipStream_t st) {
+    RoundLap lap(5);
+    const uint64_t n = p->n;
+    const HFr v = HFr::load(v_limbs);
+    const HFr &zeta = p->zeta;
+    const HFr &ba = p->bar[0], &bb = p->bar[1], &bc = p->bar[2], &bs1 = p->bar[3], &bs2 = p->bar[4], &bzw = p->bar[5];
+    const HFr w = fr_root_of_unity(p->log_n);
+    Fr* r = p->poly(P_R);
+    if (p->r_eval.active) ZCHK(eval_many_finish(p->scratch_r(), &p->r_eval, st));
+    const HFr bar_r = p->bar_r;
     const HFr v2 = v * v, v3 = v2 * v, v4 = v3 * v, v5 = v4 * v;
     std::vector<LcTerm> wt = {{r, p->r_len, HFr::one()}, {p->poly(P_AX), n + 2, v}, {p->poly(P_BX), n + 2, v2},
                               {p->poly(P_CX), n + 2, v3}, {p->circuit(C_S1), n, v4}, {p->circuit(C_S2), n, v5}};
+    host_mark(H_SCALARS);
     Fr* num = p->t;
     ZCHK(lincomb_dev(wt, num, p->r_len, st));
     ZCHK(poke_add(num, 0, (bar_r + v * ba + v2 * bb + v3 * bc + v4 * bs1 + v5 * bs2).neg(), st));
@@ -626,7 +761,7 @@
     ZCHK(poke_add(num2, 0, bzw.neg(), st));
     {
         const DivReq dv[2] = {{num, p->r_len, zeta, p->poly(P_WZ)}, {num2, n + 3, zeta * w, p->poly(P_WZW)}};
-        ZCHK(div_linear_batch_dev(p->scratch(), dv, 2, st));
+        ZCHK(div_linear_batch_dev(p->scratch(), dv, 2, st, &p->div_pre));
     }
     p->wzw_len = n + 2;
     if (p->wz_len == p->wzw_len) {
@@ -638,6 +773,14 @@
     }
     p->stage = 5;
     return ZKP_OK;
+}
+int zkp_plonk_round5(zkp_plonk_prover* p, const uint64_t v_limbs[4], uint64_t* out_xy , uint8_t* out_inf ) try {
+    if (!p || !v_limbs || !out_xy || !out_inf) return fail(ZKP_E_ARG, "null argument");
+    if (p->stage < 4) return fail(ZKP_E_ARG, "round 4 has not run");
+    CTX_ENTER(p->srs->slot);
+    hipStream_t st = nullptr;
+    WsOrder ord(st);
+    return round5_body(p, v_limbs, out_xy, out_inf, st);
 } ZKP_CATCH_INT
 
 int zkp_plonk_get_poly(zkp_plonk_prover* p, int which, uint64_t* out, size_t cap_elems, size_t* len) try {
@@ -768,6 +911,10 @@
     if (p->srs->d_inf.p) return fail(ZKP_E_ARG, "SRS with infinity points");
     if (p->para_table.empty()) ZCHK(build_para_table(p));
     std::memset(out, 0, sizeof *out);
+    CTX_ENTER(p->srs->slot);
+    hipStream_t st = nullptr;
+    WsOrder ord(st);
+    HostLap lap(0);
     PlonkChallengeGenerator ch;
     auto feed = [&](int i) {
         uint64_t x[6] = {0}, y[6] = {0};
@@ -779,18 +926,27 @@
         ch.feed(x, y, out->commit_is_inf[i] != 0);
     };
     uint64_t c2[8], c1[4];
-    ZCHK(zkp_plonk_round1(p, blinders, out->commit_xy[0], out->commit_is_inf));
+    host_mark(H_TRANSCRIPT);
+    ZCHK(round1_body(p, blinders, out->commit_xy[0], out->commit_is_inf, st));
+    host_mark(H_ENTRY);
     feed(0); feed(1); feed(2);
     ch.generate(2, c2);
-    ZCHK(zkp_plonk_round2(p, c2, c2 + 4, blinders + 24, out->commit_xy[3], out->commit_is_inf + 3));
+    host_mark(H_TRANSCRIPT);
+    ZCHK(round2_body(p, c2, c2 + 4, blinders + 24, out->commit_xy[3], out->commit_is_inf + 3, st));
+    host_mark(H_ENTRY);
     feed(3);
     ch.generate(1, c1);
     size_t degree = 0;
-    ZCHK(zkp_plonk_round3(p, c1, out->commit_xy[4], out->commit_is_inf + 4, &degree));
+    host_mark(H_TRANSCRIPT);
+    ZCHK(round3_body(p, c1, out->commit_xy[4], out->commit_is_inf + 4, &degree, st));
+    host_mark(H_ENTRY);
     out->degree = degree;
     feed(4); feed(5); feed(6);
     ch.generate(1, c1);
-    ZCHK(zkp_plonk_round4(p, c1, out->bars[0]));
+    host_mark(H_TRANSCRIPT);
+    if (!knob_flag(KNOB_POOL_NO_WARM)) host_pool().warm(std::chrono::microseconds(500));
+    ZCHK(round4_body(p, c1, out->bars[0], st));
+    host_mark(H_ENTRY);
     HXyzz para[6];
     uint64_t para_xy[6 * 12];
     uint8_t para_inf[6];
@@ -798,7 +954,9 @@
         const std::function<void(size_t)> job = [&](size_t i) { para[i] = commit_para_xyzz(p, HFr::load(out->bars[i])); };
         host_pool().run(job, 6);
     }
+    host_mark(H_PARA);
     batch_to_affine(para, 6, para_xy, para_inf);
+    host_mark(H_AFFINE);
     for (int i = 0; i < 6; i++) {
         const uint64_t* xy = para_xy + 12 * i;
         const uint8_t inf = para_inf[i];
@@ -811,8 +969,12 @@
         ch.feed(x, y, inf != 0);
     }
     ch.generate(1, c1);
-    ZCHK(zkp_plonk_round5(p, c1, out->commit_xy[7], out->commit_is_inf + 7));
+    host_mark(H_TRANSCRIPT);
+    ZCHK(round5_body(p, c1, out->commit_xy[7], out->commit_is_inf + 7, st));
+    host_mark(H_ENTRY);
     feed(7); feed(8);
     ch.generate(1, out->u);
+    host_mark(H_TRANSCRIPT);
+    lap.flush();
     return ZKP_OK;
 } ZKP_CATCH_INT
```
